# autonomousvision/LaRa

Hardware: AMD Instinct MI355X
Metric: novel-view frames/sec @512x512 (4-view in, 2DGS fwd+bwd) (higher is better)
Workload: dtype f32 raster + bf16-MFMA/f32-accumulate encoder (+ bf16-autocast coarse decoder MLP, as the reference's bf16-mixed)

## Files before the change

### lara_amd/csrc/abi.hip

```cpp
#include <stdlib.h>
#include <string.h>

#include "common.h"

static thread_local int g_last_hip_error = 0;
void l2d_set_hip_error(hipError_t e) { g_last_hip_error = (int)e; }

#include <atomic>
#include <mutex>
#include <map>
#include <utility>
#include <vector>
namespace {
struct ProfRec { const char *name; hipEvent_t a, b; };
std::atomic<bool> g_prof_on{false};
std::mutex g_prof_mu;
std::vector<ProfRec> g_prof_log;
std::vector<hipEvent_t> g_prof_pool;
hipEvent_t prof_event() {
    if (!g_prof_pool.empty()) { hipEvent_t e = g_prof_pool.back(); g_prof_pool.pop_back(); return e; }
    hipEvent_t e = nullptr;
    (void)hipEventCreate(&e);
    return e;
}
}

L2dProfScope::L2dProfScope(const char *name, hipStream_t stream) : slot(-1), s(stream) {
    if (!g_prof_on.load(std::memory_order_relaxed)) return;
    std::lock_guard<std::mutex> lk(g_prof_mu);
    ProfRec r{name, prof_event(), prof_event()};
    (void)hipEventRecord(r.a, s);
    g_prof_log.push_back(r);
    slot = (int)g_prof_log.size() - 1;
}
L2dProfScope::~L2dProfScope() {
    if (slot < 0) return;
    std::lock_guard<std::mutex> lk(g_prof_mu);
    if (slot < (int)g_prof_log.size()) (void)hipEventRecord(g_prof_log[slot].b, s);
}

namespace {

bool make_view(const lara2dgs_view *view, ViewDev &v) {
    if (!view) return false;
    if (view->P < 0 || view->image_height <= 0 || view->image_width <= 0) return false;
    if (view->sh_degree < 0 || view->sh_degree > 3) return false;
    if (view->capacity < 0 || view->capacity > 0xffffffffll) return false;
    if (!view->bg || !view->viewmatrix || !view->projmatrix || !view->campos) return false;
    v.P = view->P;
    v.deg = view->sh_degree;
    v.M = view->sh_coeffs;
    v.H = view->image_height;
    v.W = view->image_width;
    v.gx = (v.W + TILE - 1) / TILE;
    v.gy = (v.H + TILE - 1) / TILE;
    v.tiles = v.gx * v.gy;
    if (v.gx > 65535 || v.gy > 65535) return false;
    v.scale_modifier = view->scale_modifier;
    v.cull_transparent = (view->prefiltered >> 1) & 1;
    v.tight_tiles = (view->prefiltered >> 2) & 1;
    v.cap = (unsigned)view->capacity;
    v.fwd_only = view->forward_only != 0;
    v.counts_out = view->counts_out;
    {
        static const unsigned dbg = getenv("LARA2DGS_DEBUG_FLAGS") ? (unsigned)strtoul(getenv("LARA2DGS_DEBUG_FLAGS"), nullptr, 0) : 0u;
        v.dbg = dbg;
    }
    v.bg = view->bg;
    v.viewmatrix = view->viewmatrix;
    v.projmatrix = view->projmatrix;
    v.campos = view->campos;
    return true;
}

StateView carve_state(const ViewDev &v, void *state) {
    lara2dgs_state_layout L;
    state_layout(v.P, v.H, v.W, v.cap, v.fwd_only, &L);
    char *b = (char *)state;
    StateView s;
    s.header = (uint32_t *)(b + L.header);
    s.geom = (float4 *)(b + L.geom);
    s.cullbox = (float4 *)(b + L.cullbox);
    s.point_list = (uint32_t *)(b + L.point_list);
    s.ranges = (uint2 *)(b + L.ranges);
    s.tile_order = (uint32_t *)(b + L.tile_order);
    s.pair_base = (uint32_t *)(b + L.pair_base);
    s.pair_pos = (uint32_t *)(b + L.pair_pos);
    s.final_T = (float *)(b + L.final_T);
    s.n_contrib = (uint32_t *)(b + L.n_contrib);
    s.seg_base = (uint32_t *)(b + L.seg_base);
    s.seg_cnt = (uint32_t *)(b + L.seg_cnt);
    s.bwd_order = (uint32_t *)(b + L.bwd_order);
    s.bwd_items = (uint2 *)(b + L.bwd_items);
    s.ckpt = (float *)(b + L.ckpt);
    s.pair_mask = (uint2 *)(b + L.pair_mask);
    s.tile_maxc = (uint32_t *)(b + L.tile_maxc);
    s.seg_cost = (uint32_t *)(b + L.seg_cost);
    return s;
}

ScratchView carve_scratch(const ViewDev &v, void *scratch, ScratchLayout &L) {
    scratch_layout(v.P, v.H, v.W, v.cap, v.fwd_only, &L);
    char *b = (char *)scratch;
    ScratchView s;
    s.tile_count = (uint32_t *)(b + L.tile_count);
    s.tile_fill = (uint32_t *)(b + L.tile_fill);
    s.sub_start = (uint32_t *)(b + L.sub_start);
    s.sort_parts = (uint32_t *)(b + L.sort_parts);
    s.sort_items = (uint2 *)(b + L.sort_items);
    s.rect = (uint4 *)(b + L.rect);
    s.keys = (uint64_t *)(b + L.keys);
    s.block_tot = (uint32_t *)(b + L.block_tot);
    s.pair_grad = (float4 *)(b + L.pair_grad);
    s.pair_valid = (uint32_t *)(b + L.pair_valid);
    return s;
}

}

extern "C" {

int lara2dgs_abi_version(void) { return LARA2DGS_ABI_VERSION; }

const char *lara2dgs_error_string(int code) {
    switch (code) {
    case LARA2DGS_OK: return "ok";
    case LARA2DGS_E_INVALID: return "invalid argument";
    case LARA2DGS_E_LAUNCH: return "HIP launch/API failure (see lara2dgs_last_hip_error)";
    case LARA2DGS_E_UNSUPPORTED: return "unsupported configuration";
    default: return "unknown error";
    }
}

int lara2dgs_last_hip_error(void) { return g_last_hip_error; }

int64_t lara2dgs_state_bytes(int32_t P, int32_t H, int32_t W, int64_t capacity, int32_t forward_only) {
    if (P < 0 || H <= 0 || W <= 0 || capacity < 0) return LARA2DGS_E_INVALID;
    lara2dgs_state_layout L;
    state_layout(P, H, W, capacity, forward_only != 0, &L);
    return L.total;
}

int64_t lara2dgs_scratch_bytes(int32_t P, int32_t H, int32_t W, int64_t capacity, int32_t forward_only) {
    if (P < 0 || H <= 0 || W <= 0 || capacity < 0) return LARA2DGS_E_INVALID;
    ScratchLayout L;
    scratch_layout(P, H, W, capacity, forward_only != 0, &L);
    return L.total;
}

int lara2dgs_get_state_layout(int32_t P, int32_t H, int32_t W, int64_t capacity, int32_t forward_only,
                              lara2dgs_state_layout *out) {
    if (!out || P < 0 || H <= 0 || W <= 0 || capacity < 0) return LARA2DGS_E_INVALID;
    state_layout(P, H, W, capacity, forward_only != 0, out);
    return LARA2DGS_OK;
}

int lara2dgs_mark_visible(int32_t P, const float *means3D, const float *viewmatrix,
                          const float *projmatrix, uint8_t *present, void *stream) {
    (void)projmatrix;
    if (P < 0 || (P > 0 && (!means3D || !viewmatrix || !present))) return LARA2DGS_E_INVALID;
    return launch_mark_visible(P, means3D, viewmatrix, present, (hipStream_t)stream);
}

int lara2dgs_selftest(int which, const float *in, float *out, void *stream) {
    if (which != 0 || !in || !out) return LARA2DGS_E_INVALID;
    return launch_selftest_butterfly(in, out, (hipStream_t)stream);
}

int lara2dgs_profile_enable(int on) {
    g_prof_on.store(on != 0);
    return LARA2DGS_OK;
}

int lara2dgs_profile_collect(char *names, int names_len, float *ms, int max_entries) {
    std::lock_guard<std::mutex> lk(g_prof_mu);
    int n = 0, pos = 0;
    for (size_t i = 0; i < g_prof_log.size(); i++) {
        ProfRec &r = g_prof_log[i];
        if (n < max_entries && names && ms) {
            const int len = (int)strlen(r.name) + 1;
            if (pos + len <= names_len) {
                float t = 0.f;
                (void)hipEventSynchronize(r.b);
                (void)hipEventElapsedTime(&t, r.a, r.b);
                memcpy(names + pos, r.name, len);
                pos += len;
                ms[n++] = t;
            }
        }
        g_prof_pool.push_back(r.a);
        g_prof_pool.push_back(r.b);
    }
    g_prof_log.clear();
    return n;
}

}

namespace {

bool views_agree(int n, const lara2dgs_view *views) {
    for (int i = 1; i < n; i++) {
        const lara2dgs_view &a = views[0], &b = views[i];
        if (a.P != b.P || a.sh_degree != b.sh_degree || a.sh_coeffs != b.sh_coeffs || a.image_height != b.image_height ||
            a.image_width != b.image_width || a.capacity != b.capacity || a.prefiltered != b.prefiltered ||
            a.scale_modifier != b.scale_modifier || a.debug != b.debug || a.forward_only != b.forward_only) return false;
        if (b.counts_out != (a.counts_out ? a.counts_out + 4 * i : nullptr)) return false;
    }
    return true;
}

void grad_layout(int64_t P, int M, bool sh, bool col, bool sr, bool tm, lara2dgs_grad_layout *L) {
    int64_t o = 0;
    auto sec = [&](bool on, int64_t n) { if (!on) return (int64_t)-1; const int64_t at = o; o = (o + n + 3) / 4 * 4; return at; };
    L->means3D = sec(true, P * 3);
    L->means2D = sec(true, P * 3);
    L->shs = sec(sh, P * M * 3);
    L->colors = sec(col, P * 3);
    L->opacities = sec(true, P);
    L->scales = sec(sr, P * 2);
    L->rotations = sec(sr, P * 4);
    L->transmat = sec(tm, P * 9);
    L->total = o;
}

__global__ void __launch_bounds__(256) zero_strided_kernel(char *__restrict__ base, const int64_t stride, const int64_t bytes) {
    uint4 *p = (uint4 *)(base + (int64_t)blockIdx.y * stride);
    const int64_t n = bytes / 16;
    for (int64_t i = (int64_t)blockIdx.x * 256 + threadIdx.x; i < n; i += (int64_t)gridDim.x * 256) p[i] = make_uint4(0u, 0u, 0u, 0u);
}

inline int zero_strided(void *base, int64_t stride, int64_t bytes, int n_views, hipStream_t s) {
    const int64_t n = (bytes + 15) / 16;
    const unsigned gx = (unsigned)(n < 256 * 64 ? (n + 255) / 256 : 64);
    L2D_LAUNCH_IN_SCOPE(s, zero_strided_kernel, dim3(gx ? gx : 1, (unsigned)n_views), dim3(256), 0, (char *)base, stride, (bytes + 15) / 16 * 16);
    return LARA2DGS_OK;
}

bool strides_ok(const lara2dgs_view &v0, int64_t state_stride, int64_t scratch_stride) {
    return state_stride % 256 == 0 && scratch_stride % 256 == 0 &&
           state_stride >= lara2dgs_state_bytes(v0.P, v0.image_height, v0.image_width, v0.capacity, v0.forward_only) &&
           scratch_stride >= lara2dgs_scratch_bytes(v0.P, v0.image_height, v0.image_width, v0.capacity, v0.forward_only);
}

void one_view_strides(const lara2dgs_view &v, int64_t &state_stride, int64_t &scratch_stride) {
    state_stride = align_up(lara2dgs_state_bytes(v.P, v.image_height, v.image_width, v.capacity, v.forward_only), 256);
    scratch_stride = align_up(lara2dgs_scratch_bytes(v.P, v.image_height, v.image_width, v.capacity, v.forward_only), 256);
}
}

extern "C" {

int lara2dgs_get_grad_layout(int32_t P, int32_t sh_coeffs, int32_t has_shs, int32_t has_colors,
                             int32_t has_scale_rot, int32_t has_transmat, lara2dgs_grad_layout *out) {
    if (!out || P < 0 || sh_coeffs < 0) return LARA2DGS_E_INVALID;
    grad_layout(P, sh_coeffs, has_shs != 0, has_colors != 0, has_scale_rot != 0, has_transmat != 0, out);
    return LARA2DGS_OK;
}

static int forward_views_impl(int32_t n_views, const lara2dgs_view *views, const float *means3D,
                           const float *shs, const float *colors_precomp, const float *opacities,
                           const float *scales, const float *rotations, const float *transmat_precomp,
                           float *out_color, float *out_allmap, int32_t *out_radii, void *state,
                           int64_t state_stride, void *scratch, int64_t scratch_stride, void *stream,
                           const lara2dgs_subset *subset) {
    if (n_views <= 0 || !views || !state || !scratch) return LARA2DGS_E_INVALID;
    if (subset) {
        if (!subset->coarse_state || !subset->inv || subset->coarse_P < views[0].P || subset->coarse_capacity < 0 ||
            subset->coarse_capacity > 0xffffffffll || subset->coarse_state_stride % 256) return LARA2DGS_E_INVALID;
        if (!views[0].forward_only && subset->coarse_forward_only) return LARA2DGS_E_INVALID;
        if (subset->coarse_state_stride < lara2dgs_state_bytes(subset->coarse_P, views[0].image_height, views[0].image_width,
                                                                subset->coarse_capacity, subset->coarse_forward_only)) return LARA2DGS_E_INVALID;
    }
    if (!views_agree(n_views, views)) return LARA2DGS_E_INVALID;
    const lara2dgs_view &v0 = views[0];
    if (!strides_ok(v0, state_stride, scratch_stride)) return LARA2DGS_E_INVALID;
    hipStream_t caller = (hipStream_t)stream;
    const int64_t HW = (int64_t)v0.image_height * v0.image_width;
    if (!out_color || !out_allmap) return LARA2DGS_E_INVALID;
    if (v0.P > 0) {
        if (!means3D || !opacities || !out_radii) return LARA2DGS_E_INVALID;
        if ((shs == nullptr) == (colors_precomp == nullptr)) return LARA2DGS_E_INVALID;
        if ((scales && rotations) == (transmat_precomp != nullptr)) return LARA2DGS_E_INVALID;
    }
    std::vector<ViewDev> vd(n_views);
    std::vector<StateView> st(n_views);
    std::vector<ScratchView> sc(n_views);
    std::vector<int32_t *> rad(n_views);
    for (int i = 0; i < n_views; i++) {
        if (!make_view(&views[i], vd[i])) return LARA2DGS_E_INVALID;
        if (v0.P > 0 && shs && vd[i].M < (vd[i].deg + 1) * (vd[i].deg + 1)) return LARA2DGS_E_INVALID;
        st[i] = carve_state(vd[i], (char *)state + i * state_stride);
        ScratchLayout SL;
        sc[i] = carve_scratch(vd[i], (char *)scratch + i * scratch_stride, SL);
        rad[i] = out_radii + (int64_t)i * v0.P;
        if (i == 0)
            L2D_TRY(zero_strided(sc[0].tile_count, scratch_stride, SL.sub_start - SL.tile_count, n_views, caller));
    }
    int rc = LARA2DGS_OK;
    for (int i0 = 0; i0 < n_views && rc == LARA2DGS_OK; i0 += L2D_MAX_VIEWS) {
        ViewBatch vb{};
        vb.n = n_views - i0 < L2D_MAX_VIEWS ? n_views - i0 : L2D_MAX_VIEWS;
        vb.state_stride = state_stride; vb.scratch_stride = scratch_stride;
        for (int k = 0; k < vb.n; k++) vb.bg[k] = vd[i0 + k].bg;
        rc = launch_preprocess_fwd_views(vd[i0], vb.n, &vd[i0], n_views > 1, means3D, shs, colors_precomp, opacities, scales,
                                         rotations, transmat_precomp, &st[i0], &sc[i0], &rad[i0], caller);
        if (rc == LARA2DGS_OK && !subset) rc = launch_binning(vd[i0], st[i0], sc[i0], caller, vb);
        if (rc == LARA2DGS_OK && subset) {
            ViewDev cv = vd[i0];
            cv.P = subset->coarse_P; cv.cap = (unsigned)subset->coarse_capacity; cv.fwd_only = subset->coarse_forward_only != 0;
            const StateView cst = carve_state(cv, (char *)const_cast<void *>(subset->coarse_state) + (int64_t)i0 * subset->coarse_state_stride);
            rc = launch_binning_subset(vd[i0], st[i0], sc[i0], caller, vb, cst, subset->coarse_state_stride, subset->inv);
        }
        if (rc == LARA2DGS_OK)
            rc = launch_composite_fwd(vd[i0], st[i0], sc[i0], out_color + (int64_t)i0 * 3 * HW, out_allmap + (int64_t)i0 * 7 * HW,
                                      caller, vb);
    }
    return rc;
}

int lara2dgs_forward_views(int32_t n_views, const lara2dgs_view *views, const float *means3D,
                           const float *shs, const float *colors_precomp, const float *opacities,
                           const float *scales, const float *rotations, const float *transmat_precomp,
                           float *out_color, float *out_allmap, int32_t *out_radii, void *state,
                           int64_t state_stride, void *scratch, int64_t scratch_stride, void *stream) {
    return forward_views_impl(n_views, views, means3D, shs, colors_precomp, opacities, scales, rotations, transmat_precomp, out_color,
                              out_allmap, out_radii, state, state_stride, scratch, scratch_stride, stream, nullptr);
}

int lara2dgs_forward_views_subset(int32_t n_views, const lara2dgs_view *views, const float *means3D,
                                  const float *shs, const float *colors_precomp, const float *opacities,
                                  const float *scales, const float *rotations, const float *transmat_precomp,
                                  float *out_color, float *out_allmap, int32_t *out_radii, void *state,
                                  int64_t state_stride, void *scratch, int64_t scratch_stride,
                                  const lara2dgs_subset *subset, void *stream) {
    if (!subset) return LARA2DGS_E_INVALID;
    return forward_views_impl(n_views, views, means3D, shs, colors_precomp, opacities, scales, rotations, transmat_precomp, out_color,
                              out_allmap, out_radii, state, state_stride, scratch, scratch_stride, stream, subset);
}

static int backward_views_impl(int32_t n_views, const lara2dgs_view *views, const float *means3D, const float *shs,
                               const float *colors_precomp, const float *scales, const float *rotations,
                               const float *transmat_precomp, const int32_t *radii, const float *dL_dcolor,
                               const float *dL_dallmap, void *state, int64_t state_stride, void *scratch,
                               int64_t scratch_stride, float *dL_dmeans3D, float *dL_dmeans2D, float *dL_dshs,
                               float *dL_dcolors, float *dL_dopacities, float *dL_dscales, float *dL_drotations,
                               float *dL_dtransmat, void *stream) {
    const lara2dgs_view &v0 = views[0];
    hipStream_t caller = (hipStream_t)stream;
    const int64_t HW = (int64_t)v0.image_height * v0.image_width;
    std::vector<ViewDev> vd(n_views);
    std::vector<StateView> st(n_views);
    std::vector<ScratchView> sc(n_views);
    std::vector<const int32_t *> rad(n_views);
    std::vector<ScratchLayout> SL(n_views);
    for (int i = 0; i < n_views; i++) {
        if (!make_view(&views[i], vd[i])) return LARA2DGS_E_INVALID;
        st[i] = carve_state(vd[i], (char *)state + i * state_stride);
        sc[i] = carve_scratch(vd[i], (char *)scratch + i * scratch_stride, SL[i]);
        rad[i] = radii + (int64_t)i * v0.P;
    }
    int rc = LARA2DGS_OK;
    for (int i0 = 0; i0 < n_views && rc == LARA2DGS_OK; i0 += L2D_MAX_VIEWS) {
        ViewBatch vb{};
        vb.n = n_views - i0 < L2D_MAX_VIEWS ? n_views - i0 : L2D_MAX_VIEWS;
        vb.state_stride = state_stride; vb.scratch_stride = scratch_stride;
        for (int k = 0; k < vb.n; k++) vb.bg[k] = vd[i0 + k].bg;
        rc = launch_bwd_order(vd[i0], st[i0], sc[i0], caller, vb, sc[i0].pair_valid, SL[i0].total - SL[i0].pair_valid);
        if (rc == LARA2DGS_OK)
            rc = launch_composite_bwd(vd[i0], st[i0], sc[i0], dL_dcolor + (int64_t)i0 * 3 * HW, dL_dallmap ? dL_dallmap + (int64_t)i0 * 7 * HW : nullptr, caller, vb);
        if (rc == LARA2DGS_OK)
            rc = launch_preprocess_bwd_views(vd[i0], vb.n, &vd[i0], n_views > 1, i0 > 0, means3D, shs, colors_precomp, scales,
                                             rotations, transmat_precomp, &rad[i0], &st[i0], &sc[i0], dL_dmeans3D, dL_dmeans2D,
                                             dL_dshs, dL_dcolors, dL_dopacities, dL_dscales, dL_drotations, dL_dtransmat, caller);
    }
    return rc;
}

int lara2dgs_backward_views(int32_t n_views, const lara2dgs_view *views, const float *means3D,
                            const float *shs, const float *colors_precomp, const float *scales,
                            const float *rotations, const float *transmat_precomp, const int32_t *radii,
                            const float *dL_dcolor, const float *dL_dallmap, void *state,
                            int64_t state_stride, void *scratch, int64_t scratch_stride,
                            float *grad_out, void *stream) {
    if (n_views <= 0 || !views || !state || !scratch || !grad_out) return LARA2DGS_E_INVALID;
    if (!views_agree(n_views, views)) return LARA2DGS_E_INVALID;
    const lara2dgs_view &v0 = views[0];
    if (v0.forward_only) return LARA2DGS_E_INVALID;
    if (!strides_ok(v0, state_stride, scratch_stride)) return LARA2DGS_E_INVALID;
    if (!dL_dcolor) return LARA2DGS_E_INVALID;
    const bool has_sh = shs != nullptr, has_col = colors_precomp != nullptr, has_sr = scales && rotations,
               has_tm = transmat_precomp != nullptr;
    lara2dgs_grad_layout G;
    grad_layout(v0.P, v0.sh_coeffs, has_sh, has_col, has_sr, has_tm, &G);
    if (v0.P == 0 || G.total == 0) return LARA2DGS_OK;
    if (!means3D || !radii) return LARA2DGS_E_INVALID;
    if (has_sh == has_col || has_sr == has_tm) return LARA2DGS_E_INVALID;
    auto at = [&](int64_t off) { return off < 0 ? (float *)nullptr : grad_out + off; };
    return backward_views_impl(n_views, views, means3D, shs, colors_precomp, scales, rotations, transmat_precomp, radii,
                               dL_dcolor, dL_dallmap, state, state_stride, scratch, scratch_stride, at(G.means3D),
                               at(G.means2D), at(G.shs), at(G.colors), at(G.opacities), at(G.scales), at(G.rotations),
                               at(G.transmat), stream);
}

int lara2dgs_forward(const lara2dgs_view *view, const float *means3D, const float *shs,
                     const float *colors_precomp, const float *opacities, const float *scales,
                     const float *rotations, const float *transmat_precomp, float *out_color,
                     float *out_allmap, int32_t *out_radii, void *state, void *scratch,
                     void *stream) {
    ViewDev v;
    if (!make_view(view, v)) return LARA2DGS_E_INVALID;
    if (!out_color || !out_allmap || !state || !scratch) return LARA2DGS_E_INVALID;
    if (v.P > 0) {
        if (!means3D || !opacities || !out_radii) return LARA2DGS_E_INVALID;
        if ((shs == nullptr) == (colors_precomp == nullptr)) return LARA2DGS_E_INVALID;
        const bool has_sr = scales && rotations;
        if (has_sr == (transmat_precomp != nullptr)) return LARA2DGS_E_INVALID;
        if (shs && v.M < (v.deg + 1) * (v.deg + 1)) return LARA2DGS_E_INVALID;
    }
    int64_t sst, qst;
    one_view_strides(*view, sst, qst);
    return forward_views_impl(1, view, means3D, shs, colors_precomp, opacities, scales, rotations, transmat_precomp, out_color,
                              out_allmap, out_radii, state, sst, scratch, qst, stream, nullptr);
}

int lara2dgs_backward(const lara2dgs_view *view, const float *means3D, const float *shs,
                      const float *colors_precomp, const float *scales, const float *rotations,
                      const float *transmat_precomp, const int32_t *radii, const float *dL_dcolor,
                      const float *dL_dallmap, void *state, void *scratch,
                      float *dL_dmeans3D, float *dL_dmeans2D, float *dL_dshs, float *dL_dcolors,
                      float *dL_dopacities, float *dL_dscales, float *dL_drotations,
                      float *dL_dtransmat, void *stream) {
    ViewDev v;
    if (!make_view(view, v)) return LARA2DGS_E_INVALID;
    if (!dL_dcolor || !state || !scratch) return LARA2DGS_E_INVALID;
    if (v.fwd_only) return LARA2DGS_E_INVALID;
    if (v.P == 0) return LARA2DGS_OK;
    if (!means3D || !radii || !dL_dmeans3D || !dL_dmeans2D || !dL_dopacities) return LARA2DGS_E_INVALID;
    if ((shs == nullptr) == (colors_precomp == nullptr)) return LARA2DGS_E_INVALID;
    if (shs && !dL_dshs) return LARA2DGS_E_INVALID;
    if (colors_precomp && !dL_dcolors) return LARA2DGS_E_INVALID;
    const bool has_sr = scales && rotations;
    if (has_sr == (transmat_precomp != nullptr)) return LARA2DGS_E_INVALID;
    if (has_sr && (!dL_dscales || !dL_drotations)) return LARA2DGS_E_INVALID;
    if (transmat_precomp && !dL_dtransmat) return LARA2DGS_E_INVALID;
    int64_t sst, qst;
    one_view_strides(*view, sst, qst);
    return backward_views_impl(1, view, means3D, shs, colors_precomp, scales, rotations, transmat_precomp, radii, dL_dcolor,
                               dL_dallmap, state, sst, scratch, qst, dL_dmeans3D, dL_dmeans2D, dL_dshs, dL_dcolors,
                               dL_dopacities, dL_dscales, dL_drotations, dL_dtransmat, stream);
}

}
```

### lara_amd/csrc/common.h

```cpp
#pragma once
#include <hip/hip_runtime.h>
#include <stdint.h>

#include "../../include/lara2dgs.h"
#include "launch.h"

#define TILE 16
#define NEAR_N 0.2f
#define FAR_N 100.0f
#define FILTER_SIZE 0.707106f
#define FILTER_INV_SQUARE 2.0f
#define CUTOFF 3.0f
#define GEOM_F 20
#define L2D_SLICES 16
#define L2D_LDS_HIST_TILES 8192
#define GRAD_F 20
#define L2D_SEG 512
#define L2D_CKPT_F 10
#define L2D_MAX_VIEWS 8

struct ViewDev {
    int P, deg, M, H, W, gx, gy, tiles;
    float scale_modifier;
    unsigned cap;
    unsigned dbg;
    int cull_transparent;
    int tight_tiles;
    int fwd_only;
    const float *bg, *viewmatrix, *projmatrix, *campos;
    uint32_t *counts_out;
};

struct ViewBatch {
    int n;
    long long state_stride, scratch_stride;
    const float *bg[L2D_MAX_VIEWS];
};
#ifdef __HIPCC__
template <class T>
__device__ __forceinline__ T *l2d_view_ptr(T *p, const long long stride_bytes) {
    return (T *)((const char *)p + (long long)blockIdx.z * stride_bytes);
}
#endif

struct StateView {
    uint32_t *header;
    float4 *geom;
    float4 *cullbox;
    uint32_t *point_list;
    uint2 *ranges;
    uint32_t *tile_order;
    uint32_t *pair_base;
    uint32_t *pair_pos;
    float *final_T;
    uint32_t *n_contrib;
    uint32_t *seg_base;
    uint32_t *seg_cnt;
    uint32_t *bwd_order;
    uint2 *bwd_items;
    float *ckpt;
    uint2 *pair_mask;
    uint32_t *tile_maxc;
    uint32_t *seg_cost;
};

struct ScratchView {
    uint32_t *tile_count;
    uint32_t *tile_fill;
    uint32_t *sub_start;
    uint32_t *sort_parts;
    uint2 *sort_items;
    uint4 *rect;
    uint64_t *keys;
    uint32_t *block_tot;
    float4 *pair_grad;
    uint32_t *pair_valid;
};

static inline int64_t align_up(int64_t x, int64_t a) { return (x + a - 1) / a * a; }
static inline size_t up256(size_t v) { return (v + 255) & ~(size_t)255; }

__host__ __device__ static inline int64_t l2d_ckpt_slots(int64_t cap) { return cap / L2D_SEG + 1; }

static inline void state_layout(int P, int H, int W, int64_t cap, int fwd_only, lara2dgs_state_layout *L) {
    const int64_t tiles = (int64_t)((W + TILE - 1) / TILE) * ((H + TILE - 1) / TILE);
    const int64_t HW = (int64_t)H * W;
    const int64_t k = fwd_only ? 0 : 1;
    int64_t o = 0;
    L->header = o;      o = align_up(o + 256, 256);
    L->geom = o;        o = align_up(o + (int64_t)P * GEOM_F * 4, 256);
    L->cullbox = o;     o = align_up(o + (int64_t)P * 16, 256);
    L->point_list = o;  o = align_up(o + cap * 4, 256);
    L->ranges = o;      o = align_up(o + tiles * 8, 256);
    L->tile_order = o;  o = align_up(o + tiles * 4, 256);
    L->pair_base = o;   o = align_up(o + k * ((int64_t)P + 1) * 4, 256);
    L->pair_pos = o;    o = align_up(o + k * cap * 4, 256);
    L->final_T = o;     o = align_up(o + k * L2D_CKPT_F * HW * 4, 256);
    L->n_contrib = o;   o = align_up(o + k * 2 * HW * 4, 256);
    const int64_t nseg = cap / L2D_SEG + 1;
    L->seg_base = o;    o = align_up(o + k * (tiles + 1) * 4, 256);
    L->seg_cnt = o;     o = align_up(o + k * tiles * 4, 256);
    L->bwd_order = o;   o = align_up(o + k * tiles * 4, 256);
    L->bwd_items = o;   o = align_up(o + k * (nseg + tiles) * 8, 256);
    L->ckpt = o;        o = align_up(o + k * l2d_ckpt_slots(cap) * L2D_CKPT_F * 256 * 4, 256);
    L->pair_mask = o;   o = align_up(o + k * cap * 8, 256);
    L->tile_maxc = o;   o = align_up(o + k * tiles * 4, 256);
    L->seg_cost = o;    o = align_up(o + k * (nseg + tiles) * 4, 256);
    L->total = o;
}

struct ScratchLayout { int64_t tile_count, tile_fill, sub_start, sort_parts, sort_items, rect, keys, block_tot, pair_grad, pair_valid, total; };
static inline void scratch_layout(int P, int H, int W, int64_t cap, int fwd_only, ScratchLayout *L) {
    const int64_t tiles = (int64_t)((W + TILE - 1) / TILE) * ((H + TILE - 1) / TILE);
    int64_t o = 0;
    L->tile_count = o;  o = align_up(o + tiles * 4 * L2D_SLICES, 256);
    L->tile_fill = o;   o = align_up(o + tiles * 4 * L2D_SLICES, 256);
    L->sub_start = o;   o = align_up(o + tiles * 4 * L2D_SLICES, 256);
    L->sort_parts = o;  o = align_up(o + (tiles + 1) * 4, 256);
    L->sort_items = o;  o = align_up(o + tiles * 8, 256);
    const int64_t fwd0 = o;
    L->rect = o;        o = align_up(o + (int64_t)P * 16, 256);
    L->keys = o;        o = align_up(o + cap * 8, 256);
    L->block_tot = o;   o = align_up(o + (((int64_t)P + 255) / 256 + 1) * 4, 256);
    const int64_t fwd_end = o;
    L->pair_grad = fwd0;
    L->pair_valid = align_up(fwd0 + cap * GRAD_F * 4, 256);
    const int64_t bwd_end = align_up(L->pair_valid + cap + 256, 256);
    L->total = (fwd_only || fwd_end > bwd_end) ? fwd_end : bwd_end;
}

int launch_preprocess_fwd_views(const ViewDev &v, int n, const ViewDev *views, bool multi, const float *means3D, const float *shs,
                                const float *colors_precomp, const float *opacities, const float *scales,
                                const float *rotations, const float *transmat_precomp, const StateView *st,
                                const ScratchView *sc, int32_t *const *radii, hipStream_t s);
int launch_binning(const ViewDev &v, StateView st, ScratchView sc, hipStream_t s, const ViewBatch &vb);
int launch_binning_subset(const ViewDev &v, StateView st, ScratchView sc, hipStream_t s, const ViewBatch &vb, StateView cst,
                          long long coarse_stride, const int32_t *inv);
int launch_composite_fwd(const ViewDev &v, StateView st, ScratchView sc, float *out_color, float *out_allmap,
                         hipStream_t s, const ViewBatch &vb);
int launch_bwd_order(const ViewDev &v, StateView st, ScratchView sc, hipStream_t s, const ViewBatch &vb, void *zero_base, int64_t zero_bytes);
int launch_composite_bwd(const ViewDev &v, StateView st, ScratchView sc, const float *dL_dcolor,
                         const float *dL_dallmap, hipStream_t s, const ViewBatch &vb);
int launch_preprocess_bwd_views(const ViewDev &v, int n, const ViewDev *views, bool multi, int accumulate, const float *means3D,
                                const float *shs, const float *colors_precomp, const float *scales, const float *rotations,
                                const float *transmat_precomp, const int32_t *const *radii, const StateView *st,
                                const ScratchView *sc, float *dL_dmeans3D, float *dL_dmeans2D, float *dL_dshs,
                                float *dL_dcolors, float *dL_dopacities, float *dL_dscales, float *dL_drotations,
                                float *dL_dtransmat, hipStream_t s);
int launch_selftest_butterfly(const float *in, float *out, hipStream_t s);
int launch_mark_visible(int P, const float *means3D, const float *viewmatrix, uint8_t *present,
                        hipStream_t s);
```

### lara_amd/csrc/composite.hip

```cpp
#include "common.h"
#include "tilebox.h"
#include "wave.h"

namespace {

constexpr int FWD_CHUNK = 512;
constexpr int REC4 = 6;

__device__ __forceinline__ void cross3(const float a[3], const float b[3], float o[3]) {
    o[0] = a[1] * b[2] - a[2] * b[1];
    o[1] = a[2] * b[0] - a[0] * b[2];
    o[2] = a[0] * b[1] - a[1] * b[0];
}

template <int CHUNK>
__device__ __forceinline__ uint32_t stage_entry(const float4 *__restrict__ geom, const uint32_t id,
                                                const float4 cb, const bool valid, const float X0,
                                                const float Y0, float4 *rec, uint32_t *ids,
                                                const int e = threadIdx.x, uint2 *mask_out = nullptr) {
    float4 r0 = make_float4(0.f, 0.f, 0.f, 0.f), r1 = r0, r2 = r0, r3 = r0, r4 = r0, r5 = r0;
    uint32_t mask_lo = 0, mask_hi = 0, rectpack = 0;
    int gx0 = 0, gx1 = -1, gy0 = 0, gy1 = -1;
    if (valid) {
        l2d_box_cells<2>(cb.x, cb.y, X0, 8.f, gx0, gx1);
        l2d_box_cells<2>(cb.z, cb.w, Y0, 8.f, gy0, gy1);
    }
    if (gx0 <= gx1 && gy0 <= gy1) {
        const float4 *g = geom + (size_t)id * 5;
        const float4 g0 = g[0], g1 = g[1], g2 = g[2], g3 = g[3], g4 = g[4];
        const float Tu[3] = {g0.x, g0.y, g0.z}, Tv[3] = {g0.w, g1.x, g1.y}, Tw[3] = {g1.z, g1.w, g2.x};
        const float k0[3] = {X0 * Tw[0] - Tu[0], X0 * Tw[1] - Tu[1], X0 * Tw[2] - Tu[2]};
        const float l0[3] = {Y0 * Tw[0] - Tv[0], Y0 * Tw[1] - Tv[1], Y0 * Tw[2] - Tv[2]};
        float A[3], B[3], C[3];
        cross3(k0, l0, A);
        cross3(Tw, l0, B);
        cross3(k0, Tw, C);
        const float cx = g2.y - X0, cy = g2.z - Y0, opa = g2.w;
        const float tau = 2.0f * __logf(255.0f * opa) * 1.001f + 0.01f;
        const float nb = B[0] * B[0] + B[1] * B[1], qa = nb - tau * B[2] * B[2];
        const bool ellipse = qa > 1e-5f * (nb + tau * B[2] * B[2]);
        const float inv_qa = ellipse ? __builtin_amdgcn_rcpf(qa) : 0.f;
        const float bx0 = (float)(2 * gx0), bx1 = (float)(2 * gx1 + 1);
        uint32_t colsum = 0;
        for (int by = gy0; by <= gy1; by++) {
            float lo = 1e9f, hi = -1e9f;
#pragma unroll
            for (int q = 0; q < 2; q++) {
                const float y = (float)(2 * by + q);
                const float u0 = A[0] + y * C[0], u1 = A[1] + y * C[1], u2 = A[2] + y * C[2];
                const float qb = u0 * B[0] + u1 * B[1] - tau * (u2 * B[2]);
                const float qc = u0 * u0 + u1 * u1 - tau * (u2 * u2);
                const float disc = qb * qb - qa * qc + 4e-6f * (qb * qb);
                if (!ellipse) {
                    lo = bx0; hi = bx1;
                } else if (disc >= 0.f) {
                    const float sq = __builtin_amdgcn_sqrtf(disc);
                    lo = fminf(lo, (-qb - sq) * inv_qa);
                    hi = fmaxf(hi, (-qb + sq) * inv_qa);
                }
                const float h = 0.5f * tau - (y - cy) * (y - cy);
                if (h >= 0.f) {
                    const float sh = __builtin_amdgcn_sqrtf(h);
                    lo = fminf(lo, cx - sh);
                    hi = fmaxf(hi, cx + sh);
                }
            }
            const int ilo = (int)ceilf(fmaxf(lo - 0.02f, bx0)), ihi = (int)floorf(fminf(hi + 0.02f, bx1));
            if (ilo <= ihi) {
                const uint32_t cols = ((2u << (ihi >> 1)) - 1u) & ~((1u << (ilo >> 1)) - 1u);
                colsum |= cols;
                if (by < 4) mask_lo |= cols << (8 * by);
                else mask_hi |= cols << (8 * (by - 4));
            }
        }
        if (colsum) {
            const int rx0 = __builtin_ctz(colsum), rx1 = 31 - __builtin_clz(colsum);
            const int ry0 = mask_lo ? (__builtin_ctz(mask_lo) >> 3) : 4 + (__builtin_ctz(mask_hi) >> 3);
            const int ry1 = mask_hi ? 4 + ((31 - __builtin_clz(mask_hi)) >> 3) : ((31 - __builtin_clz(mask_lo)) >> 3);
            rectpack = (uint32_t)rx0 | ((uint32_t)rx1 << 4) | ((uint32_t)ry0 << 8) | ((uint32_t)ry1 << 12) | (1u << 16);
            r0 = make_float4(A[0], A[1], A[2], B[0]);
            r1 = make_float4(B[1], B[2], C[0], C[1]);
            r2 = make_float4(C[2], cx, cy, Tw[0]);
            r3 = make_float4(Tw[1], Tw[2], opa, __uint_as_float(mask_lo));
            r4 = make_float4(g3.x, g3.y, g3.z, g4.x);
            r5 = make_float4(g4.y, g4.z, __uint_as_float(mask_hi), 0.f);
        }
    }
    rec[0 * CHUNK + e] = r0; rec[1 * CHUNK + e] = r1; rec[2 * CHUNK + e] = r2;
    rec[3 * CHUNK + e] = r3; rec[4 * CHUNK + e] = r4; rec[5 * CHUNK + e] = r5;
    if (ids) ids[e] = valid ? id : 0u;
    if (mask_out && valid) *mask_out = make_uint2(mask_lo, mask_hi);
    return rectpack;
}

template <int CHUNK>
__device__ __forceinline__ void stage_entry_masked(const float4 *__restrict__ geom, const uint32_t id, const uint2 mask,
                                                   const bool valid, const float X0, const float Y0, float4 *rec,
                                                   uint32_t *ids, const int e) {
    float4 r0 = make_float4(0.f, 0.f, 0.f, 0.f), r1 = r0, r2 = r0, r3 = r0, r4 = r0, r5 = r0;
    if (valid && (mask.x | mask.y)) {
        const float4 *g = geom + (size_t)id * 5;
        const float4 g0 = g[0], g1 = g[1], g2 = g[2], g3 = g[3], g4 = g[4];
        const float Tu[3] = {g0.x, g0.y, g0.z}, Tv[3] = {g0.w, g1.x, g1.y}, Tw[3] = {g1.z, g1.w, g2.x};
        const float k0[3] = {X0 * Tw[0] - Tu[0], X0 * Tw[1] - Tu[1], X0 * Tw[2] - Tu[2]};
        const float l0[3] = {Y0 * Tw[0] - Tv[0], Y0 * Tw[1] - Tv[1], Y0 * Tw[2] - Tv[2]};
        float A[3], B[3], C[3];
        cross3(k0, l0, A);
        cross3(Tw, l0, B);
        cross3(k0, Tw, C);
        r0 = make_float4(A[0], A[1], A[2], B[0]);
        r1 = make_float4(B[1], B[2], C[0], C[1]);
        r2 = make_float4(C[2], g2.y - X0, g2.z - Y0, Tw[0]);
        r3 = make_float4(Tw[1], Tw[2], g2.w, __uint_as_float(mask.x));
        r4 = make_float4(g3.x, g3.y, g3.z, g4.x);
        r5 = make_float4(g4.y, g4.z, __uint_as_float(mask.y), 0.f);
    }
    rec[0 * CHUNK + e] = r0; rec[1 * CHUNK + e] = r1; rec[2 * CHUNK + e] = r2;
    rec[3 * CHUNK + e] = r3; rec[4 * CHUNK + e] = r4; rec[5 * CHUNK + e] = r5;
    ids[e] = valid ? id : 0u;
}

struct Hit {
    float sx, sy, rz, depth, G, alpha, ddx, ddy;
    bool use3d;
};

struct EntryRec { float4 r0, r1, r2, r3; };
template <int CHUNK>
__device__ __forceinline__ EntryRec load_entry(const float4 *rec, const int j) {
    EntryRec e;
    e.r0 = rec[0 * CHUNK + j]; e.r1 = rec[1 * CHUNK + j]; e.r2 = rec[2 * CHUNK + j]; e.r3 = rec[3 * CHUNK + j];
    return e;
}

__device__ __forceinline__ bool eval_rec(const EntryRec &e, const float lx, const float ly, Hit &h,
                                         float Tw[3], float &opa) {
    const float4 r0 = e.r0, r1 = e.r1, r2 = e.r2, r3 = e.r3;
    const float px = r0.x + lx * r0.w + ly * r1.z;
    const float py = r0.y + lx * r1.x + ly * r1.w;
    const float pz = r0.z + lx * r1.y + ly * r2.x;
    Tw[0] = r2.w; Tw[1] = r3.x; Tw[2] = r3.y; opa = r3.z;
    h.rz = __builtin_amdgcn_rcpf(pz);
    h.sx = px * h.rz; h.sy = py * h.rz;
    const float rho3d = h.sx * h.sx + h.sy * h.sy;
    h.ddx = r2.y - lx; h.ddy = r2.z - ly;
    const float rho2d = FILTER_INV_SQUARE * (h.ddx * h.ddx + h.ddy * h.ddy);
    h.use3d = rho3d <= rho2d;
    const float rho = fminf(rho3d, rho2d);
    h.depth = h.use3d ? (h.sx * Tw[0] + h.sy * Tw[1]) + Tw[2] : Tw[2];
    const float power = -0.5f * rho;
    h.G = __expf(power);
    h.alpha = fminf(0.99f, opa * h.G);
    return (pz != 0.0f) & (h.depth >= NEAR_N) & !(power > 0.0f) & !(h.alpha < 1.0f / 255.0f);
}

__device__ __forceinline__ unsigned long long quad_masks(const uint32_t bm, const int qx4, const int grp) {
    unsigned long long m = 0ull;
#pragma unroll
    for (int g = 0; g < 16; g++) {
        const int bit = (g >> 2) * 8 + qx4 + (g & 3);
        const unsigned long long b = __ballot((bm >> bit) & 1u);
        m = (grp == g) ? b : m;
    }
    return m;
}

struct FwdPixel {
    float T = 1.0f, C0 = 0.f, C1 = 0.f, C2 = 0.f, N0 = 0.f, N1 = 0.f, N2 = 0.f;
    float Dd = 0.f, M1 = 0.f, M2 = 0.f, distortion = 0.f, median_depth = 0.f;
    uint32_t last_contributor = 0, median_contributor = 0;
    bool done = false;

    template <int CHUNK>
    __device__ __forceinline__ void blend(const float4 *rec, const int j, const int base, bool valid,
                                          const Hit &h) {
        valid = valid && !done;
        const float test_T = T * (1.0f - h.alpha);
        const bool kill = valid && test_T < 0.0001f;
        done = done || kill;
        valid = valid && !kill;
        if (__ballot(valid) == 0ull) return;
        const float4 r4 = rec[4 * CHUNK + j], r5 = rec[5 * CHUNK + j];
        const float a = valid ? h.alpha : 0.f;
        const float depth = valid ? h.depth : 1.0f;
        const float w = a * T;
        const float A = 1.0f - T;
        const float mm = FAR_N / (FAR_N - NEAR_N) * (1.0f - NEAR_N * __builtin_amdgcn_rcpf(depth));
        distortion += (mm * mm * A + M2 - 2.0f * mm * M1) * w;
        Dd += depth * w;
        M1 += mm * w;
        M2 += mm * mm * w;
        const bool med = valid && T > 0.5f;
        median_depth = med ? depth : median_depth;
        median_contributor = med ? (uint32_t)(base + j + 1) : median_contributor;
        N0 += r4.x * w; N1 += r4.y * w; N2 += r4.z * w;
        C0 += r4.w * w; C1 += r5.x * w; C2 += r5.y * w;
        T = valid ? test_T : T;
        last_contributor = valid ? (uint32_t)(base + j + 1) : last_contributor;
    }

};

template <bool KEEP>
__global__ void __launch_bounds__(256)
composite_fwd_kernel(ViewDev v, const uint32_t *__restrict__ header, const uint2 *__restrict__ ranges,
                     const uint32_t *__restrict__ point_list, const float4 *__restrict__ geom,
                     const uint32_t *__restrict__ tile_order, const float4 *__restrict__ cullbox,
                     float *__restrict__ final_T, uint32_t *__restrict__ n_contrib,
                     const uint32_t *__restrict__ seg_base, const uint32_t *__restrict__ seg_cnt,
                     float *__restrict__ ckpt, uint2 *__restrict__ pair_mask, uint32_t *__restrict__ tile_maxc,
                     uint32_t *__restrict__ seg_cost,
                     float *__restrict__ out_color, float *__restrict__ out_allmap, const ViewBatch vb) {
    {
        const long long sst = vb.state_stride, HWb = (long long)v.H * v.W * 4;
        header = l2d_view_ptr(header, sst); ranges = l2d_view_ptr(ranges, sst); point_list = l2d_view_ptr(point_list, sst);
        geom = l2d_view_ptr(geom, sst); tile_order = l2d_view_ptr(tile_order, sst); cullbox = l2d_view_ptr(cullbox, sst);
        final_T = l2d_view_ptr(final_T, sst); n_contrib = l2d_view_ptr(n_contrib, sst); seg_base = l2d_view_ptr(seg_base, sst);
        seg_cnt = l2d_view_ptr(seg_cnt, sst); ckpt = l2d_view_ptr(ckpt, sst); pair_mask = l2d_view_ptr(pair_mask, sst);
        tile_maxc = l2d_view_ptr(tile_maxc, sst); seg_cost = l2d_view_ptr(seg_cost, sst);
        out_color = l2d_view_ptr(out_color, 3 * HWb); out_allmap = l2d_view_ptr(out_allmap, 7 * HWb);
        v.bg = vb.bg[blockIdx.z];
    }
    constexpr int CHUNK = FWD_CHUNK;
    static_assert(L2D_SEG % FWD_CHUNK == 0, "segment boundaries must fall on round boundaries");
    __shared__ float4 rec[REC4 * CHUNK];
    __shared__ unsigned long long qmask[4][16][CHUNK / 64];
    uint32_t &s_cost = *(uint32_t *)&rec[5 * CHUNK + 0].w;
    uint32_t &s_tmax = *(uint32_t *)&rec[5 * CHUNK + 1].w;
    uint32_t &s_ndone = *(uint32_t *)&rec[5 * CHUNK + 2].w;
    const int tile = (v.dbg & 8u) ? (int)blockIdx.x : (int)tile_order[blockIdx.x];
    const int tx = tile % v.gx, ty = tile / v.gx;
    const int wave = threadIdx.x >> 6, lane = threadIdx.x & 63;
    const int grp = lane >> 2;
    const int lxi = (wave & 1) * 8 + (grp & 3) * 2 + (lane & 1);
    const int lyi = (wave >> 1) * 8 + (grp >> 2) * 2 + ((lane >> 1) & 1);
    const int pxi = tx * TILE + lxi, pyi = ty * TILE + lyi;
    const bool inside = pxi < v.W && pyi < v.H;
    const size_t HW = (size_t)v.H * v.W;
    const size_t pix = (size_t)pyi * v.W + pxi;
    const float lx = (float)lxi, ly = (float)lyi;
    const float X0 = (float)(tx * TILE), Y0 = (float)(ty * TILE);

    if (header[1]) {
        if (inside) {
            const float qnan = __uint_as_float(0x7fc00000u);
            for (int ch = 0; ch < 3; ch++) out_color[ch * HW + pix] = qnan;
            for (int ch = 0; ch < 7; ch++) out_allmap[ch * HW + pix] = qnan;
            if (KEEP) {
                for (int ch = 0; ch < L2D_CKPT_F; ch++) final_T[pix + ch * HW] = qnan;
                n_contrib[pix] = 0; n_contrib[pix + HW] = 0;
            }
        }
        return;
    }

    const uint2 range = ranges[tile];
    const int total = (int)(range.y - range.x);
    const int lo = 0, hi = total;
    FwdPixel px;
    px.done = !inside;
    uint32_t *dbg_hdr = const_cast<uint32_t *>(header);
    const long long dbg_t0 = (v.dbg & 32u) ? (long long)__builtin_readcyclecounter() : 0ll;
    int dbg_rounds = 0;

    const int tid = threadIdx.x;
    const uint32_t cost_nb = KEEP ? seg_cnt[tile] : 0u;
    uint32_t *const cost_full = KEEP ? seg_cost + seg_base[tile] : nullptr,
             *const cost_last = KEEP ? seg_cost + (v.cap / L2D_SEG + 1u) + tile : nullptr;
    if (KEEP)
        for (uint32_t q = tid; q <= cost_nb; q += 256) *(q < cost_nb ? cost_full + q : cost_last) = 0u;
    int cost_round = -1;
    constexpr int SPT = CHUNK / 256;
    uint32_t id1[SPT], id2[SPT];
    float4 cb1[SPT];
#pragma unroll
    for (int q = 0; q < SPT; q++) {
        const int o = lo + q * 256 + tid;
        id1[q] = o < hi ? point_list[range.x + o] : 0u;
        id2[q] = CHUNK + o < hi ? point_list[range.x + CHUNK + o] : 0u;
    }
#pragma unroll
    for (int q = 0; q < SPT; q++) cb1[q] = lo + q * 256 + tid < hi ? cullbox[id1[q]] : make_float4(0.f, 0.f, 0.f, 0.f);
    if (threadIdx.x < 3) *(uint32_t *)&rec[5 * CHUNK + threadIdx.x].w = 0u;
    __syncthreads();
    for (int base = lo; base < hi; base += CHUNK) {
        {
            const bool wave_done = __ballot(px.done) == ~0ull;
            if (wave_done && lane == 0) atomicAdd(&s_ndone, 1u);
            __syncthreads();
            if (s_ndone == 4u) break;
        }
        if (KEEP && tid == 0) {
            if (cost_round >= 0) { if ((uint32_t)cost_round < cost_nb) cost_full[cost_round] = s_cost; else *cost_last += s_cost; }
            s_cost = 0u;
        }
        cost_round = (base - lo) / CHUNK;
        dbg_rounds++;
        if (KEEP && base && base % L2D_SEG == 0 && !px.done) {
            float *ck = ckpt + ((size_t)seg_base[tile] + (size_t)(base / L2D_SEG - 1)) * (L2D_CKPT_F * 256) + tid;
            ck[0 * 256] = px.T; ck[1 * 256] = px.M1; ck[2 * 256] = px.M2;
            ck[3 * 256] = px.C0; ck[4 * 256] = px.C1; ck[5 * 256] = px.C2;
            ck[6 * 256] = px.Dd; ck[7 * 256] = px.N0; ck[8 * 256] = px.N1; ck[9 * 256] = px.N2;
        }
#pragma unroll
        for (int q = 0; q < SPT; q++) {
            const int o = q * 256 + tid;
            const uint32_t id0 = id1[q];
            const float4 cb0 = cb1[q];
            id1[q] = id2[q];
            id2[q] = base + 2 * CHUNK + o < hi ? point_list[range.x + base + 2 * CHUNK + o] : 0u;
            cb1[q] = base + CHUNK + o < hi ? cullbox[id1[q]] : make_float4(0.f, 0.f, 0.f, 0.f);
            stage_entry<CHUNK>(geom, id0, cb0, base + o < hi, X0, Y0, rec, nullptr, o,
                               KEEP && base + o < hi ? pair_mask + range.x + base + o : nullptr);
        }
        __syncthreads();
        if (__ballot(!px.done) == 0ull) continue;
        const int nw = (min(CHUNK, hi - base) + 63) >> 6;
        unsigned long long *qm = &qmask[wave][grp][0];
#pragma unroll 1
        for (int w = 0; w < nw; w++) {
            const float4 *mrec = rec + ((wave >> 1) ? 5 : 3) * CHUNK + w * 64 + lane;
            const uint32_t bm = __float_as_uint((wave >> 1) ? mrec->z : mrec->w);
            unsigned long long m = 0ull;
            if (__ballot((bm & (0x0f0f0f0fu << ((wave & 1) * 4))) != 0u) != 0ull) m = quad_masks(bm, (wave & 1) * 4, grp);
            if ((lane & 3) == 0) qm[w] = m;
        }
        int w = 0;
        unsigned long long mm = qm[0];
        if (((__ballot(px.done) >> (lane & ~3)) & 0xfull) == 0xfull) { mm = 0ull; w = nw; }
        auto next = [&](bool &has, int &j) {
            while (mm == 0ull && w + 1 < nw) { w++; mm = qm[w]; }
            has = mm != 0ull;
            j = has ? 64 * w + __builtin_ctzll(mm) : 0;
            mm &= mm - 1ull;
        };
        bool hA0, hA1, hB0 = false, hB1 = false;
        int jA0, jA1, jB0 = 0, jB1 = 0;
        next(hA0, jA0);
        next(hA1, jA1);
        EntryRec rA0 = load_entry<CHUNK>(rec, jA0), rA1 = load_entry<CHUNK>(rec, jA1), rB0, rB1;
        auto trip = [&](const EntryRec &c0, const EntryRec &c1, const int j0, const int j1, const bool has0, const bool has1,
                        EntryRec &x0, EntryRec &x1, int &k0, int &k1, bool &n0, bool &n1) {
            next(n0, k0);
            next(n1, k1);
            x0 = load_entry<CHUNK>(rec, k0);
            x1 = load_entry<CHUNK>(rec, k1);
            Hit h0, h1;
            float Tw0[3], Tw1[3], opa0, opa1;
            const bool e0 = eval_rec(c0, lx, ly, h0, Tw0, opa0) && has0;
            const bool e1 = eval_rec(c1, lx, ly, h1, Tw1, opa1) && has1;
            if (v.dbg & 4u) {
                atomicAdd(&dbg_hdr[4], ((lane & 3) == 0) ? (unsigned)has0 + (unsigned)has1 : 0u);
                atomicAdd(&dbg_hdr[5], (unsigned)e0 + (unsigned)e1);
                if (lane == 0) atomicAdd(&dbg_hdr[6], 1u);
            }
            px.blend<CHUNK>(rec, j0, base, e0, h0);
            px.blend<CHUNK>(rec, j1, base, e1, h1);
            if (((__ballot(px.done) >> (lane & ~3)) & 0xfull) == 0xfull) { mm = 0ull; w = nw; n0 = false; n1 = false; }
        };
        uint32_t ntrips = 0;
        while (true) {
            if (__ballot(hA0) == 0ull) break;
            trip(rA0, rA1, jA0, jA1, hA0, hA1, rB0, rB1, jB0, jB1, hB0, hB1);
            ntrips++;
            if (__ballot(hB0) == 0ull) break;
            trip(rB0, rB1, jB0, jB1, hB0, hB1, rA0, rA1, jA0, jA1, hA0, hA1);
            ntrips++;
        }
        if (KEEP && lane == 0 && ntrips) atomicAdd(&s_cost, ntrips);
    }
    const float T = px.T;
    if (KEEP) {
        if (threadIdx.x == 0) s_tmax = 0u;
        __syncthreads();
        uint32_t m = px.last_contributor;
#pragma unroll
        for (int d = 1; d < 64; d <<= 1) m = max(m, (uint32_t)__shfl_xor((int)m, d, 64));
        if (lane == 0) atomicMax(&s_tmax, m);
        __syncthreads();
        if (threadIdx.x == 0) {
            tile_maxc[tile] = s_tmax;
            if (cost_round >= 0) { if ((uint32_t)cost_round < cost_nb) cost_full[cost_round] = s_cost; else *cost_last += s_cost; }
        }
    }
    if (inside) {
        if (KEEP) {
            final_T[pix] = T;
            final_T[pix + HW] = px.M1;
            final_T[pix + 2 * HW] = px.M2;
            final_T[pix + 3 * HW] = px.C0; final_T[pix + 4 * HW] = px.C1; final_T[pix + 5 * HW] = px.C2;
            final_T[pix + 6 * HW] = px.Dd;
            final_T[pix + 7 * HW] = px.N0; final_T[pix + 8 * HW] = px.N1; final_T[pix + 9 * HW] = px.N2;
            n_contrib[pix] = px.last_contributor;
            n_contrib[pix + HW] = px.median_contributor;
        }
        out_color[0 * HW + pix] = px.C0 + T * v.bg[0];
        out_color[1 * HW + pix] = px.C1 + T * v.bg[1];
        out_color[2 * HW + pix] = px.C2 + T * v.bg[2];
        out_allmap[0 * HW + pix] = px.Dd;
        out_allmap[1 * HW + pix] = 1.0f - T;
        out_allmap[2 * HW + pix] = px.N0;
        out_allmap[3 * HW + pix] = px.N1;
        out_allmap[4 * HW + pix] = px.N2;
        out_allmap[5 * HW + pix] = px.median_depth;
        out_allmap[6 * HW + pix] = px.distortion;
        if ((v.dbg & 32u) && lane == 0) {
            out_allmap[6 * HW + pix] = (float)((long long)__builtin_readcyclecounter() - dbg_t0);
            out_allmap[5 * HW + pix] = (float)dbg_rounds;
        }
    }
}

__device__ __forceinline__ float mul_legacy(const float a, const float b) {
    float r;
    asm("v_mul_legacy_f32 %0, %1, %2" : "=v"(r) : "v"(a), "v"(b));
    return r;
}

struct QuadCoef { float a1, a2, a3, b1, b2, b3; };
__device__ __forceinline__ QuadCoef quad_coef(const int lane, const float lx, const float ly) {
    QuadCoef k;
    const int l = lane & 3;
    k.a1 = l == 0 ? 1.f : (l == 1 ? lx - 1.f : (l == 2 ? ly : 0.f));
    k.a2 = l == 1 ? 1.f : 0.f;
    k.a3 = l == 3 ? 1.f : 0.f;
    k.b1 = l == 0 ? ly : (l == 2 ? 1.f : (l == 3 ? lx - 1.f : 0.f));
    k.b2 = l == 3 ? 1.f : 0.f;
    k.b3 = l == 1 ? 1.f : 0.f;
    return k;
}
__device__ __forceinline__ void quad_reduce_scatter(const float dp[3], const float q[3], const float h[10], const QuadCoef &k,
                                                    float r[6], const int lane) {
    const bool b0 = lane & 1, b1 = lane & 2;
#pragma unroll
    for (int c = 0; c < 3; c++) {
        float d = dp[c];
        asm volatile("" : "+v"(d));
        const float t = d + dpp_move<0xB1, 0xf>(d);
        const float tq = q[c] + dpp_move<0xB1, 0xf>(q[c]);
        const float mine = k.a1 * t + (k.a2 * d + k.a3 * tq);
        const float send = k.b1 * t + (k.b2 * d + k.b3 * tq);
        r[c] = mine + dpp_move<0x4E, 0xf>(send);
    }
    float v1[5];
#pragma unroll
    for (int i = 0; i < 5; i++) {
        const float mine = b0 ? h[2 * i + 1] : h[2 * i];
        const float send = b0 ? h[2 * i] : h[2 * i + 1];
        v1[i] = mine + dpp_move<0xB1, 0xf>(send);
    }
#pragma unroll
    for (int i = 0; i < 2; i++) {
        const float mine = b1 ? v1[2 * i + 1] : v1[2 * i];
        const float send = b1 ? v1[2 * i] : v1[2 * i + 1];
        r[3 + i] = mine + dpp_move<0x4E, 0xf>(send);
    }
    r[5] = v1[4] + dpp_move<0x4E, 0xf>(v1[4]);
}
__device__ __forceinline__ void quad_reduce_scatter16(const float dp[3], const float q[3], const float h[4], const QuadCoef &k,
                                                      float r[4], const int lane) {
    const bool b0 = lane & 1, b1 = lane & 2;
#pragma unroll
    for (int c = 0; c < 3; c++) {
        float d = dp[c], qq = q[c];
        asm volatile("" : "+v"(d));
        asm volatile("" : "+v"(qq));
        const float t = d + dpp_move<0xB1, 0xf>(d);
        const float tq = qq + dpp_move<0xB1, 0xf>(qq);
        const float mine = k.a1 * t + (k.a2 * d + k.a3 * tq);
        const float send = k.b1 * t + (k.b2 * d + k.b3 * tq);
        r[c] = mine + dpp_move<0x4E, 0xf>(send);
    }
    float v1[2];
#pragma unroll
    for (int i = 0; i < 2; i++) {
        const float mine = b0 ? h[2 * i + 1] : h[2 * i];
        const float send = b0 ? h[2 * i] : h[2 * i + 1];
        v1[i] = mine + dpp_move<0xB1, 0xf>(send);
    }
    const float mine = b1 ? v1[1] : v1[0];
    const float send = b1 ? v1[0] : v1[1];
    r[3] = mine + dpp_move<0x4E, 0xf>(send);
}

constexpr int SLAB_WIN = 128;
constexpr int SLAB_CHUNK = 128;
constexpr int SLAB_POOL = 374;
constexpr int SLAB_F = 24;
constexpr int SLAB_F_COLOR = 16;
constexpr int SLAB_POOL_COLOR = SLAB_POOL * SLAB_F / SLAB_F_COLOR;

template <bool MAPS>
__global__ void __launch_bounds__(256)
composite_bwd_kernel(ViewDev v, const uint32_t *__restrict__ header, const uint2 *__restrict__ ranges,
                     const uint32_t *__restrict__ point_list, const float4 *__restrict__ geom,
                     const uint32_t *__restrict__ tile_order, const float4 *__restrict__ cullbox,
                     const float *__restrict__ final_T, const uint32_t *__restrict__ n_contrib,
                     const uint32_t *__restrict__ seg_base, const uint32_t *__restrict__ seg_cnt,
                     const uint32_t *__restrict__ bwd_order,
                     const uint2 *__restrict__ bwd_items, const float *__restrict__ ckpt,
                     const uint2 *__restrict__ pair_mask, const uint32_t *__restrict__ tile_maxc,
                     const float *__restrict__ dL_dcolor, const float *__restrict__ dL_dallmap,
                     const uint32_t *__restrict__ pair_pos,
                     float4 *__restrict__ pair_grad, uint8_t *__restrict__ pair_valid, const ViewBatch vb) {
    {
        const long long sst = vb.state_stride, qst = vb.scratch_stride, HWb = (long long)v.H * v.W * 4;
        header = l2d_view_ptr(header, sst); ranges = l2d_view_ptr(ranges, sst); point_list = l2d_view_ptr(point_list, sst);
        geom = l2d_view_ptr(geom, sst); tile_order = l2d_view_ptr(tile_order, sst); cullbox = l2d_view_ptr(cullbox, sst);
        final_T = l2d_view_ptr(final_T, sst); n_contrib = l2d_view_ptr(n_contrib, sst); seg_base = l2d_view_ptr(seg_base, sst);
        seg_cnt = l2d_view_ptr(seg_cnt, sst); bwd_order = l2d_view_ptr(bwd_order, sst); bwd_items = l2d_view_ptr(bwd_items, sst);
        ckpt = l2d_view_ptr(ckpt, sst); pair_mask = l2d_view_ptr(pair_mask, sst); pair_pos = l2d_view_ptr(pair_pos, sst);
        tile_maxc = l2d_view_ptr(tile_maxc, sst);
        pair_grad = l2d_view_ptr(pair_grad, qst); pair_valid = l2d_view_ptr(pair_valid, qst);
        dL_dcolor = l2d_view_ptr(dL_dcolor, 3 * HWb); dL_dallmap = l2d_view_ptr(dL_dallmap, 7 * HWb);
        v.bg = vb.bg[blockIdx.z];
    }
    constexpr int WIN = SLAB_WIN;
    constexpr int POOL = MAPS ? SLAB_POOL : SLAB_POOL_COLOR, SF = MAPS ? SLAB_F : SLAB_F_COLOR;
    __shared__ float4 rec[REC4 * WIN];
    __shared__ __attribute__((aligned(16))) float pool[(POOL + 1) * SF];
    __shared__ uint16_t s_base_[2][SLAB_CHUNK];
    __shared__ unsigned long long s_live_[2][SLAB_CHUNK];
    __shared__ uint32_t s_ql[64];
    __shared__ uint32_t s_id_[2][WIN];
    __shared__ uint2 s_mask[WIN];
    __shared__ int s_nfit_[2];
    __shared__ uint32_t s_total_[2];
    if (header[1]) return;
    const unsigned long long dbg_t0 = (v.dbg & 32u) ? wall_clock64() : 0ull;
    int dbg_rounds = 0;
    uint32_t dbg_windows = 0, dbg_trips = 0, dbg_entries = 0, dbg_slots = 0, dbg_rows = 0;
    unsigned long long dbg_tp = 0ull;
    uint32_t dbg_ph[5] = {0u, 0u, 0u, 0u, 0u};
#define DBG_PHASE(k) do { if (v.dbg & 64u) { const unsigned long long t__ = __builtin_readcyclecounter(); dbg_ph[k] += (uint32_t)(t__ - dbg_tp); dbg_tp = t__; } } while (0)
    if (v.dbg & 64u) dbg_tp = __builtin_readcyclecounter();
    const uint32_t n_full = header[3];
    int tile, seg;
    if (header[22]) {
        if (blockIdx.x >= n_full + (uint32_t)v.tiles) return;
        const uint2 it = bwd_items[blockIdx.x];
        tile = (int)it.x; seg = (int)it.y;
    } else if (blockIdx.x < n_full) {
        const uint2 it = bwd_items[blockIdx.x];
        tile = (int)it.x; seg = (int)it.y;
    } else if (blockIdx.x - n_full < (uint32_t)v.tiles) {
        tile = (int)bwd_order[blockIdx.x - n_full];
        seg = (int)seg_cnt[tile];
    } else {
        return;
    }
    const uint2 range = ranges[tile];
    const int seg_lo = seg * L2D_SEG;
    const int seg_hi = seg == (int)seg_cnt[tile] ? (int)(range.y - range.x) : seg_lo + L2D_SEG;
    const int total = min((int)tile_maxc[tile], seg_hi);
    const int lo = seg_lo;
    if (total <= lo) return;
    const int tx = tile % v.gx, ty = tile / v.gx;
    const int tid = threadIdx.x, wave = tid >> 6, lane = tid & 63;
    const int grp = lane >> 2;
    const int lxi = (wave & 1) * 8 + (grp & 3) * 2 + (lane & 1);
    const int lyi = (wave >> 1) * 8 + (grp >> 2) * 2 + ((lane >> 1) & 1);
    const int pxi = tx * TILE + lxi, pyi = ty * TILE + lyi;
    const bool inside = pxi < v.W && pyi < v.H;
    const size_t HW = (size_t)v.H * v.W;
    const size_t pix = inside ? (size_t)pyi * v.W + pxi : 0;
    const float lx = (float)lxi, ly = (float)lyi;
    const float X0 = (float)(tx * TILE), Y0 = (float)(ty * TILE);

    const float T_final = inside ? final_T[pix] : 0.f;
    float T = T_final;
    const uint32_t last_contributor = inside ? n_contrib[pix] : 0u;
    const uint32_t median_contributor = (MAPS && inside) ? n_contrib[pix + HW] : 0u;
    float dpix[3] = {0.f, 0.f, 0.f}, dnrm[3] = {0.f, 0.f, 0.f};
    float dL_ddepth = 0.f, dL_daccum = 0.f, dL_dmedian = 0.f, dL_dreg = 0.f;
    float final_D = 0.f, final_D2 = 0.f;
    if (inside) {
        for (int ch = 0; ch < 3; ch++) dpix[ch] = dL_dcolor[ch * HW + pix];
        if constexpr (MAPS) {
            dL_ddepth = dL_dallmap[0 * HW + pix];
            dL_daccum = dL_dallmap[1 * HW + pix];
            for (int ch = 0; ch < 3; ch++) dnrm[ch] = dL_dallmap[(2 + ch) * HW + pix];
            dL_dmedian = dL_dallmap[5 * HW + pix];
            dL_dreg = dL_dallmap[6 * HW + pix];
            final_D = final_T[pix + HW];
            final_D2 = final_T[pix + 2 * HW];
        }
    }
    const float final_A = 1.0f - T_final;
    const float bg_dot_dpixel = v.bg[0] * dpix[0] + v.bg[1] * dpix[1] + v.bg[2] * dpix[2];

    float accum_g = 0.f, last_g = 0.f, last_alpha = 0.f;
    float last_dL_dT = 0.f;

    const int my_blk = (lyi >> 1) * 8 + (lxi >> 1);
    const uint32_t below_lo = my_blk >= 32 ? 0xffffffffu : (1u << my_blk) - 1u;
    const uint32_t below_hi = my_blk >= 32 ? (1u << (my_blk - 32)) - 1u : 0u;
    const QuadCoef qcoef = quad_coef(lane, lx, ly);
    uint32_t quad_last = last_contributor;
    quad_last = max(quad_last, (uint32_t)__builtin_amdgcn_update_dpp(0, (int)quad_last, 0xB1, 0xf, 0xf, false));
    quad_last = max(quad_last, (uint32_t)__builtin_amdgcn_update_dpp(0, (int)quad_last, 0x4E, 0xf, 0xf, false));
    if ((lane & 3) == 0) s_ql[my_blk] = quad_last;
    if (tid < SF) pool[POOL * SF + tid] = 0.f;

    if ((int)last_contributor > seg_hi) {
        const float *ck = ckpt + ((size_t)seg_base[tile] + (size_t)seg) * (L2D_CKPT_F * 256) + tid;
        const float Tb = ck[0], inv_Tb = 1.0f / Tb;
        T = Tb;
        const float s_alpha = (Tb - T_final) * inv_Tb;
        if constexpr (MAPS) {
            const float s_m1 = (final_D - ck[1 * 256]) * inv_Tb, s_m2 = (final_D2 - ck[2 * 256]) * inv_Tb;
            float sg = (Tb - T_final) * dL_daccum + (final_T[pix + 6 * HW] - ck[6 * 256]) * dL_ddepth;
            for (int ch = 0; ch < 3; ch++)
                sg += (final_T[pix + (3 + ch) * HW] - ck[(3 + ch) * 256]) * dpix[ch] +
                      (final_T[pix + (7 + ch) * HW] - ck[(7 + ch) * 256]) * dnrm[ch];
            accum_g = sg * inv_Tb;
            last_dL_dT = (final_D2 * s_alpha + final_A * s_m2 - 2.0f * final_D * s_m1) * dL_dreg;
        } else {
            (void)s_alpha;
            float sg = 0.f;
            for (int ch = 0; ch < 3; ch++) {
                float p = (final_T[pix + (3 + ch) * HW] - ck[(3 + ch) * 256]) * dpix[ch];
                asm volatile("" : "+v"(p));
                sg += p;
            }
            accum_g = sg * inv_Tb;
        }
    }

    const int se = tid - 128;
    const bool stager = se >= 0;
    uint32_t id1 = 0u, id2 = 0u;
    uint2 mk1 = make_uint2(0u, 0u), mk2 = mk1;
    auto size_round = [&](const int whi_, const int wcnt_, const int s0_, const int buf, const bool side) {
        unsigned long long *const live_ = s_live_[buf];
        uint16_t *const base_ = s_base_[buf];
                const int jm = max(whi_ - s0_ - (int)s_ql[lane], 0);
                unsigned long long la = ~0ull, lb = ~0ull;
                if (__ballot(jm > 0) != 0ull) {
                    volatile unsigned long long *vlive = live_;
                    vlive[2 * lane] = 0ull;
                    vlive[2 * lane + 1] = 0ull;
                    if (jm < SLAB_CHUNK) atomicOr(&live_[jm], 1ull << lane);
                    __builtin_amdgcn_wave_barrier();
                    la = vlive[2 * lane];
                    lb = la | vlive[2 * lane + 1];
                    unsigned long long ex = lb;
#pragma unroll
                    for (int d = 1; d < 64; d <<= 1) {
                        const uint32_t ylo = __shfl_up((uint32_t)ex, d, 64), yhi = __shfl_up((uint32_t)(ex >> 32), d, 64);
                        if (lane >= d) ex |= ((unsigned long long)yhi << 32) | ylo;
                    }
                    const uint32_t plo = __shfl_up((uint32_t)ex, 1, 64), phi = __shfl_up((uint32_t)(ex >> 32), 1, 64);
                    const unsigned long long before = lane ? (((unsigned long long)phi << 32) | plo) : 0ull;
                    la |= before; lb |= before;
                }
                uint32_t c[2];
#pragma unroll
                for (int q = 0; q < 2; q++) {
                    const int slot = s0_ + 2 * lane + q;
                    unsigned long long mk = 0ull;
                    if (slot < wcnt_) {
                        const uint2 mw = side ? s_mask[slot] : make_uint2(__float_as_uint(rec[3 * WIN + slot].w), __float_as_uint(rec[5 * WIN + slot].z));
                        mk = (((unsigned long long)mw.y << 32) | mw.x) & (q ? lb : la);
                    }
                    live_[2 * lane + q] = mk;
                    c[q] = (uint32_t)__builtin_popcountll(mk);
                }
                uint32_t incl = c[0] + c[1];
#pragma unroll
                for (int d = 1; d < 64; d <<= 1) {
                    const uint32_t y = __shfl_up(incl, d, 64);
                    if (lane >= d) incl += y;
                }
                const uint32_t b0 = incl - c[0] - c[1], b1 = incl - c[1];
                const unsigned long long f0 = __ballot(s0_ + 2 * lane < wcnt_ && b1 <= (uint32_t)POOL);
                const unsigned long long f1 = __ballot(s0_ + 2 * lane + 1 < wcnt_ && incl <= (uint32_t)POOL);
                const int L = f1 == ~0ull ? 64 : __builtin_ctzll(~f1);
                if (lane == 0) s_nfit_[buf] = L == 64 ? 128 : 2 * L + (int)((f0 >> L) & 1ull);
                base_[2 * lane] = (uint16_t)b0;
                base_[2 * lane + 1] = (uint16_t)b1;
                if (lane == 63) s_total_[buf] = incl;
    };
    {
        const int wcnt = min(WIN, total - lo);
        if (stager) {
            const uint32_t id0 = total - 1 - se >= lo ? point_list[range.x + total - 1 - se] : 0u;
            const uint2 mk0 = total - 1 - se >= lo ? pair_mask[range.x + total - 1 - se] : make_uint2(0u, 0u);
            id1 = total - WIN - 1 - se >= lo ? point_list[range.x + total - WIN - 1 - se] : 0u;
            mk1 = total - WIN - 1 - se >= lo ? pair_mask[range.x + total - WIN - 1 - se] : make_uint2(0u, 0u);
            id2 = total - 2 * WIN - 1 - se >= lo ? point_list[range.x + total - 2 * WIN - 1 - se] : 0u;
            mk2 = total - 2 * WIN - 1 - se >= lo ? pair_mask[range.x + total - 2 * WIN - 1 - se] : make_uint2(0u, 0u);
            stage_entry_masked<WIN>(geom, id0, mk0, se < wcnt, X0, Y0, rec, s_id_[0], se);
        }
        __syncthreads();
        if (wave == 3) size_round(total, wcnt, 0, 0, false);
        __syncthreads();
        DBG_PHASE(0);
    }
    int cur = 0, wb = 0;
    for (int whi = total; whi > lo; whi -= WIN) {
        const int wcnt = min(WIN, whi - lo);
        const bool more_windows = whi - WIN > lo;
        dbg_windows++;
        if (stager) s_mask[se] = mk1;
        unsigned long long wm0 = 0ull, wm1 = 0ull;

        for (int s0 = 0; s0 < wcnt;) {
            dbg_rounds++;
            const unsigned long long *const s_live = s_live_[cur];
            const uint16_t *const s_base = s_base_[cur];
            const uint32_t *const s_id = s_id_[wb];
            const int nfit = s_nfit_[cur];
            if (v.dbg & 512u) { dbg_entries += (uint32_t)nfit; dbg_slots += nfit < SLAB_CHUNK ? (uint32_t)s_base[nfit] : min(s_total_[cur], (uint32_t)POOL); }

            {
                if (s0 == 0) {
#pragma unroll
                    for (int k = 0; k < 2; k++) {
                        const float4 *mrec = rec + ((wave >> 1) ? 5 : 3) * WIN + 64 * k + lane;
                        const uint32_t bm = __float_as_uint((wave >> 1) ? mrec->z : mrec->w);
                        unsigned long long m = 0ull;
                        if (__ballot((bm & (0x0f0f0f0fu << ((wave & 1) * 4))) != 0u) != 0ull) m = quad_masks(bm, (wave & 1) * 4, grp);
                        if (k == 0) wm0 = m; else wm1 = m;
                    }
                }
                unsigned long long m0 = wm0, m1 = wm1;
                {
                    int sh = s0;
                    if (sh >= 64) { m0 = m1; m1 = 0ull; sh -= 64; }
                    if (sh) { m0 = (m0 >> sh) | (m1 << (64 - sh)); m1 >>= sh; }
                    if (nfit < 64) { m0 &= (1ull << nfit) - 1ull; m1 = 0ull; }
                    else if (nfit < 128) m1 &= (1ull << (nfit - 64)) - 1ull;
                }
                const int jmin = whi - s0 - (int)quad_last;
                if (jmin > 0) {
                    m0 = jmin >= 64 ? 0ull : m0 & (~0ull << jmin);
                    m1 = jmin >= 128 ? 0ull : (jmin > 64 ? m1 & (~0ull << (jmin - 64)) : m1);
                }
                uint32_t mm = (uint32_t)m0, q1 = (uint32_t)(m0 >> 32), q2 = (uint32_t)m1, q3 = (uint32_t)(m1 >> 32);
                int jb = 0;
                auto trip = [&]() __attribute__((always_inline)) {
                    dbg_trips++;
                    while (mm == 0u && (q1 | q2 | q3) != 0u) { mm = q1; q1 = q2; q2 = q3; q3 = 0u; jb += 32; }
                    const bool has = mm != 0u;
                    const int j = jb + (has ? __builtin_ctz(mm) : 0);
                    mm &= mm - 1u;
                    const int ws = s0 + j;
                    const uint32_t contributor = (uint32_t)(whi - 1 - ws);
                    const EntryRec ent = load_entry<WIN>(rec, ws);
                    Hit h;
                    float Tw[3], opa;
                    const bool active = eval_rec(ent, lx, ly, h, Tw, opa) && has && contributor < last_contributor;
                    const float4 r4 = rec[4 * WIN + ws], r5 = rec[5 * WIN + ws];
                    const float nrm[3] = {r4.x, r4.y, r4.z}, rgb[3] = {r4.w, r5.x, r5.y};
                    if constexpr (!MAPS) {
                        (void)nrm;
                        const float alpha = active ? h.alpha : 0.f;
                        const float inv_1ma = __builtin_amdgcn_rcpf(1.f - alpha);
                        const float T_new = T * inv_1ma;
                        const float w = alpha * T_new;
                        const float gval = __builtin_fmaf(rgb[2], dpix[2], __builtin_fmaf(rgb[0], dpix[0], rgb[1] * dpix[1]));
                        const float accum_new = mul_legacy(last_alpha, last_g) + (1.f - last_alpha) * accum_g;
                        float dL_dalpha = gval - accum_new;
                        dL_dalpha = __builtin_fmaf(T_new, dL_dalpha, -((T_final * inv_1ma) * bg_dot_dpixel));
                        T = T_new;
                        accum_g = accum_new;
                        last_g = gval;
                        last_alpha = alpha;
                        const float da = active ? dL_dalpha : 0.f;
                        const float sx = h.sx, sy = h.sy;
                        const float rz3 = (active && h.use3d) ? h.rz : 0.f;
                        const float qG = opa * da * h.G;
                        const float dL_dsx = -mul_legacy(qG, sx), dL_dsy = -mul_legacy(qG, sy);
                        const float dpx = dL_dsx * rz3, dpy = dL_dsy * rz3;
                        const float dpv[3] = {dpx, dpy, -(mul_legacy(dpx, sx) + mul_legacy(dpy, sy))};
                        const float qG2 = h.use3d ? 0.f : -FILTER_INV_SQUARE * qG;
                        const float q3[3] = {h.G * da, qG2 * h.ddx, qG2 * h.ddy};
                        const float h4[4] = {w * dpix[0], w * dpix[1], w * dpix[2], w};
                        float r[4];
                        quad_reduce_scatter16(dpv, q3, h4, qcoef, r, lane);
#pragma unroll
                        for (int i = 0; i < 4; i++) asm volatile("" : "+v"(r[i]));
                        const unsigned long long lv = s_live[has ? j : 0];
                        const int rank = __builtin_popcount((uint32_t)lv & below_lo) + __builtin_popcount((uint32_t)(lv >> 32) & below_hi);
                        float4 *ps = (float4 *)(pool + ((int)s_base[has ? j : 0] + rank) * SF) + (lane & 3);
                        if (has) *ps = make_float4(r[0], r[1], r[2], r[3]);
                    } else {
                    const float alpha = active ? h.alpha : 0.f, c_d = h.depth;
                    const float inv_1ma = __builtin_amdgcn_rcpf(1.f - alpha);
                    const float T_new = T * inv_1ma;
                    const float w = alpha * T_new;
                    const float gval = rgb[0] * dpix[0] + rgb[1] * dpix[1] + rgb[2] * dpix[2] +
                                       nrm[0] * dnrm[0] + nrm[1] * dnrm[1] + nrm[2] * dnrm[2] +
                                       c_d * dL_ddepth + dL_daccum;
                    const float accum_new = mul_legacy(last_alpha, last_g) + (1.f - last_alpha) * accum_g;
                    float dL_dalpha = gval - accum_new;
                    float dL_dz = 0.0f;
                    const float inv_cd = __builtin_amdgcn_rcpf(c_d);
                    const float m_d = FAR_N / (FAR_N - NEAR_N) * (1.f - NEAR_N * inv_cd);
                    const float dmd_dd = (FAR_N * NEAR_N) / (FAR_N - NEAR_N) * inv_cd * inv_cd;
                    if (contributor + 1 == median_contributor) dL_dz += dL_dmedian;
                    const float dL_dweight = (final_D2 + m_d * m_d * final_A - 2.f * m_d * final_D) * dL_dreg;
                    dL_dalpha += dL_dweight - last_dL_dT;
                    const float dLdT_new = mul_legacy(alpha, dL_dweight) + (1.f - alpha) * last_dL_dT;
                    const float dL_dmd = 2.0f * (T_new * alpha) * (m_d * final_A - final_D) * dL_dreg;
                    dL_dz += dL_dmd * dmd_dd;
                    dL_dalpha *= T_new;
                    dL_dalpha += (-T_final * inv_1ma) * bg_dot_dpixel;
                    dL_dz += w * dL_ddepth;
                    T = T_new;
                    accum_g = accum_new;
                    last_g = gval;
                    last_alpha = alpha;
                    last_dL_dT = dLdT_new;
                    const float ww = w, da = active ? dL_dalpha : 0.f, dz = active ? dL_dz : 0.f;
                    const float sx = h.sx, sy = h.sy;
                    const float rz3 = (active && h.use3d) ? h.rz : 0.f;
                    const float qv[3] = {mul_legacy(dz, sx), mul_legacy(dz, sy), dz};
                    const float qG = opa * da * h.G;
                    const float dL_dsx = dz * Tw[0] - mul_legacy(qG, sx);
                    const float dL_dsy = dz * Tw[1] - mul_legacy(qG, sy);
                    const float dpx = dL_dsx * rz3, dpy = dL_dsy * rz3;
                    const float dpv[3] = {dpx, dpy, -(mul_legacy(dpx, sx) + mul_legacy(dpy, sy))};
                    const float qG2 = h.use3d ? 0.f : -FILTER_INV_SQUARE * qG;
                    const float hv[10] = {qG2 * h.ddx, qG2 * h.ddy, ww * dnrm[0], ww * dnrm[1], ww * dnrm[2], h.G * da,
                                          ww * dpix[0], ww * dpix[1], ww * dpix[2], ww};
                    float r[6];
                    quad_reduce_scatter(dpv, qv, hv, qcoef, r, lane);
#pragma unroll
                    for (int i = 0; i < 6; i++) asm volatile("" : "+v"(r[i]));
                    const unsigned long long lv = s_live[has ? j : 0];
                    const int rank = __builtin_popcount((uint32_t)lv & below_lo) + __builtin_popcount((uint32_t)(lv >> 32) & below_hi);
                    float *ps = pool + ((int)s_base[has ? j : 0] + rank) * SLAB_F + (lane & 3);
                    if (has) {
                        ps[0] = r[0]; ps[4] = r[1]; ps[8] = r[2]; ps[12] = r[3]; ps[16] = r[4];
                        if (!(lane & 2)) ps[20] = r[5];
                    }
                    }
                };
                while (__ballot((mm | q1 | q2 | q3) != 0u) != 0ull) {
                    trip();
                    if (__ballot((mm | q1 | q2 | q3) != 0u) == 0ull) break;
                    trip();
                }
            }
            __syncthreads();
            DBG_PHASE(3);

            if ((wave << 5) < nfit && !(v.dbg & 2u)) {
                const int e = tid >> 1, part = tid & 1;
                const int ws = min(s0 + e, WIN - 1);
                const bool has = e < nfit;
                const int cnt = has ? __builtin_popcountll(s_live[e]) : 0;
                float4 gq0 = make_float4(0.f, 0.f, 0.f, 0.f), gq1 = gq0, gq2 = gq0;
                if (cnt && part == 0) {
                    const float4 *gm = geom + (size_t)s_id[ws] * 5;
                    gq0 = gm[0]; gq1 = gm[1]; gq2 = gm[2];
                }
                constexpr int NG = MAPS ? 22 : 16;
                float g[NG];
                const float4 *ps = (const float4 *)(pool + (int)s_base[e] * SF);
                {
                    const float4 *p0 = part < cnt ? ps + part * (SF / 4) : (const float4 *)(pool + POOL * SF);
#pragma unroll
                    for (int q = 0; q < NG / 4; q++) {
                        const float4 t = p0[q];
                        g[4 * q] = t.x; g[4 * q + 1] = t.y; g[4 * q + 2] = t.z; g[4 * q + 3] = t.w;
                    }
                    if constexpr (MAPS) {
                        const float2 t2 = *(const float2 *)(p0 + 5);
                        g[20] = t2.x; g[21] = t2.y;
                    }
                }
                for (int i = part + 2; i < cnt; i += 2) {
#pragma unroll
                    for (int q = 0; q < NG / 4; q++) {
                        const float4 t = ps[i * (SF / 4) + q];
                        g[4 * q] += t.x; g[4 * q + 1] += t.y; g[4 * q + 2] += t.z; g[4 * q + 3] += t.w;
                    }
                    if constexpr (MAPS) {
                        const float2 t2 = *(const float2 *)(ps + i * (SF / 4) + 5);
                        g[20] += t2.x; g[21] += t2.y;
                    }
                }
#pragma unroll
                for (int k = 0; k < NG; k++) g[k] += dpp_move<0xB1, 0xf>(g[k]);
                const bool touched = (MAPS ? g[21] : g[15]) > 0.f;
                if (part == 0 && touched) {
                    const uint32_t p = range.x + (uint32_t)(whi - 1 - ws);
                    const float4 g0 = gq0, g1 = gq1, g2 = gq2;
                    const float Tu[3] = {g0.x, g0.y, g0.z}, Tv[3] = {g0.w, g1.x, g1.y}, Tw[3] = {g1.z, g1.w, g2.x};
                    const float k0[3] = {X0 * Tw[0] - Tu[0], X0 * Tw[1] - Tu[1], X0 * Tw[2] - Tu[2]};
                    const float l0[3] = {Y0 * Tw[0] - Tv[0], Y0 * Tw[1] - Tv[1], Y0 * Tw[2] - Tv[2]};
                    const float a[3] = {g[0], MAPS ? g[4] : g[1], MAPS ? g[8] : g[2]};
                    const float b[3] = {MAPS ? g[1] : g[4], g[5], MAPS ? g[9] : g[6]};
                    const float cc[3] = {MAPS ? g[2] : g[8], MAPS ? g[6] : g[9], g[10]};
                    const float qd[3] = {MAPS ? g[3] : 0.f, MAPS ? g[7] : 0.f, MAPS ? g[11] : 0.f};
                    float t1[3], t2[3], dk0[3], dl0[3], dTw[3];
                    cross3(l0, a, t1); cross3(Tw, cc, t2);
                    for (int i = 0; i < 3; i++) dk0[i] = t1[i] + t2[i];
                    cross3(a, k0, t1); cross3(b, Tw, t2);
                    for (int i = 0; i < 3; i++) dl0[i] = t1[i] + t2[i];
                    cross3(l0, b, t1); cross3(cc, k0, t2);
                    for (int i = 0; i < 3; i++) {
                        dTw[i] = t1[i] + t2[i] + X0 * dk0[i] + Y0 * dl0[i];
                        if constexpr (MAPS) dTw[i] += qd[i];
                    }
                    const uint32_t q = pair_pos[p];
                    float4 *row = pair_grad + (size_t)q * (GRAD_F / 4);
                    row[0] = make_float4(-dk0[0], -dk0[1], -dk0[2], -dl0[0]);
                    row[1] = make_float4(-dl0[1], -dl0[2], dTw[0], dTw[1]);
                    if constexpr (MAPS) {
                        row[2] = make_float4(dTw[2], g[12], g[13], g[14]);
                        row[3] = make_float4(g[15], g[16], g[17], g[18]);
                        row[4] = make_float4(g[19], g[20], 0.f, 0.f);
                    } else {
                        row[2] = make_float4(dTw[2], g[13], g[14], 0.f);
                        row[3] = make_float4(0.f, 0.f, g[12], g[3]);
                        row[4] = make_float4(g[7], g[11], 0.f, 0.f);
                    }
                    pair_valid[q] = 1;
                    dbg_rows++;
                }
            }
            const bool last_round = s0 + nfit >= wcnt;
            if (stager && last_round && more_windows) {
                stage_entry_masked<WIN>(geom, id1, mk1, se < min(WIN, whi - WIN - lo), X0, Y0, rec, s_id_[wb ^ 1], se);
                id1 = id2;
                mk1 = mk2;
                id2 = whi - 3 * WIN - 1 - se >= lo ? point_list[range.x + whi - 3 * WIN - 1 - se] : 0u;
                mk2 = whi - 3 * WIN - 1 - se >= lo ? pair_mask[range.x + whi - 3 * WIN - 1 - se] : make_uint2(0u, 0u);
            }
            if (wave == 3) {
                if (!last_round) size_round(whi, wcnt, s0 + nfit, cur ^ 1, false);
                else if (more_windows) size_round(whi - WIN, min(WIN, whi - WIN - lo), 0, cur ^ 1, true);
            }
            __syncthreads();
            DBG_PHASE(4);
            s0 += nfit;
            cur ^= 1;
        }
        wb ^= 1;
    }
    if ((v.dbg & 64u) && tid == 0) {
        DBG_PHASE(4);
        uint32_t *h = const_cast<uint32_t *>(header);
        for (int k = 0; k < 5; k++) atomicAdd(&h[16 + k], dbg_ph[k] >> 6);
    }
    if (v.dbg & 512u) {
        uint32_t *h = const_cast<uint32_t *>(header);
        if (tid == 0) {
            atomicAdd(&h[24], 1u); atomicAdd(&h[25], dbg_windows); atomicAdd(&h[26], (uint32_t)dbg_rounds);
            atomicAdd(&h[28], dbg_entries); atomicAdd(&h[29], dbg_slots);
        }
        if (lane == 0) atomicAdd(&h[27], dbg_trips);
        if (dbg_rows) atomicAdd(&h[30], dbg_rows);
    }
    if ((v.dbg & 32u) && tid == 0) {
        uint32_t *h = const_cast<uint32_t *>(header);
        const unsigned long long t1 = wall_clock64();
        atomicMax(&h[8], (uint32_t)(t1 - dbg_t0));
        atomicMax((unsigned long long *)&h[12], ((unsigned long long)(uint32_t)(t1 - dbg_t0) << 32) |
                                                    ((unsigned long long)dbg_rounds << 16) | (unsigned long long)blockIdx.x);
        atomicAdd(&h[9], (uint32_t)(t1 - dbg_t0));
        atomicMax(&h[10], ~(uint32_t)dbg_t0);
        atomicMax(&h[11], (uint32_t)t1);
    }
}

__global__ void __launch_bounds__(64)
selftest_butterfly_kernel(const float *__restrict__ in, float *__restrict__ out) {
    const int lane = threadIdx.x, q4 = lane & 3, grp = lane >> 2;
    const float lx = (float)((grp & 3) * 2 + (lane & 1)), ly = (float)((grp >> 2) * 2 + ((lane >> 1) & 1));
    float dp[3], q[3], h[10], r[6];
    for (int k = 0; k < 3; k++) { dp[k] = in[lane * 16 + k]; q[k] = in[lane * 16 + 3 + k]; }
    for (int k = 0; k < 10; k++) h[k] = in[lane * 16 + 6 + k];
    quad_reduce_scatter(dp, q, h, quad_coef(lane, lx, ly), r, lane);
    float *dst = out + (lane >> 2) * 24 + q4;
    for (int i = 0; i < 5; i++) dst[4 * i] = r[i];
    if (q4 < 2) dst[20] = r[5];
}

constexpr int BO_PER_THREAD = 17;
__global__ void __launch_bounds__(1024)
bwd_order_kernel(ViewDev v, uint32_t *__restrict__ header, uint2 *__restrict__ bwd_items, const uint32_t *__restrict__ seg_cnt,
                 const uint32_t *__restrict__ seg_cost, const long long sst, char *__restrict__ zero_base, const long long zero_bytes,
                 const long long qst) {
    if (blockIdx.x >= 1) {
        uint4 *z = (uint4 *)l2d_view_ptr(zero_base, qst);
        const long long n16 = zero_bytes / 16;
        for (long long i = (long long)(blockIdx.x - 1) * 1024 + threadIdx.x; i < n16; i += (long long)(gridDim.x - 1) * 1024)
            z[i] = make_uint4(0u, 0u, 0u, 0u);
        return;
    }
    header = l2d_view_ptr(header, sst); bwd_items = l2d_view_ptr(bwd_items, sst); seg_cnt = l2d_view_ptr(seg_cnt, sst);
    seg_cost = l2d_view_ptr(seg_cost, sst);
    __shared__ uint32_t bcnt[64];
    if (header[1] || (v.dbg & 256u)) return;
    const int tid = threadIdx.x, lane = tid & 63;
    if (header[22]) return;
    const uint32_t n_full = header[3], n = n_full + (uint32_t)v.tiles;
    if (n > (uint32_t)(BO_PER_THREAD * 1024)) return;
    const uint32_t *cost_last = seg_cost + (v.cap / L2D_SEG + 1u);
    if (tid < 64) bcnt[tid] = 0u;
    __syncthreads();
    uint2 item[BO_PER_THREAD];
    uint32_t bkt[BO_PER_THREAD];
#pragma unroll
    for (int k = 0; k < BO_PER_THREAD; k++) {
        const uint32_t i = (uint32_t)tid + 1024u * k;
        bkt[k] = 64u;
        if (i < n) {
            uint32_t c;
            if (i < n_full) { item[k] = bwd_items[i]; c = seg_cost[i]; }
            else { const uint32_t t = i - n_full; item[k] = make_uint2(t, seg_cnt[t]); c = cost_last[t]; }
            bkt[k] = 63u - min(63u, c >> 2);
            atomicAdd(&bcnt[bkt[k]], 1u);
        }
    }
    __syncthreads();
    if (tid < 64) {
        const uint32_t c = bcnt[tid];
        uint32_t x = c;
#pragma unroll
        for (int d = 1; d < 64; d <<= 1) {
            const uint32_t y = __shfl_up(x, d, 64);
            if (lane >= d) x += y;
        }
        bcnt[tid] = x - c;
    }
    __syncthreads();
#pragma unroll
    for (int k = 0; k < BO_PER_THREAD; k++)
        if (bkt[k] < 64u) bwd_items[atomicAdd(&bcnt[bkt[k]], 1u)] = item[k];
    if (tid == 0) header[22] = 1u;
}

}

int launch_composite_fwd(const ViewDev &v, StateView st, ScratchView sc, float *out_color, float *out_allmap,
                         hipStream_t s, const ViewBatch &vb) {
    (void)sc;
    const unsigned nz = (unsigned)vb.n;
    {
        L2D_PROF(v.fwd_only ? "composite_fwd_only" : "composite_fwd", s);
        auto kern = v.fwd_only ? composite_fwd_kernel<false> : composite_fwd_kernel<true>;
        L2D_LAUNCH_IN_SCOPE(s, kern, dim3(v.tiles, 1, nz), dim3(256), 0, v, st.header, st.ranges, st.point_list,
                            (const float4 *)st.geom, st.tile_order, (const float4 *)st.cullbox, st.final_T, st.n_contrib, st.seg_base,
                            st.seg_cnt, st.ckpt, st.pair_mask, st.tile_maxc, st.seg_cost, out_color, out_allmap, vb);
    }
    return LARA2DGS_OK;
}

int launch_bwd_order(const ViewDev &v, StateView st, ScratchView sc, hipStream_t s, const ViewBatch &vb, void *zero_base, int64_t zero_bytes) {
    (void)sc;
    L2D_PROF("bwd_order", s);
    const int64_t zb = (zero_bytes + 15) / 16 * 16;
    const unsigned zw = zb > 0 ? (unsigned)((zb / 16 + 8191) / 8192 < 128 ? (zb / 16 + 8191) / 8192 : 128) : 0u;
    L2D_LAUNCH_IN_SCOPE(s, bwd_order_kernel, dim3(1 + zw, 1, (unsigned)vb.n), dim3(1024), 0, v, st.header, st.bwd_items, st.seg_cnt,
                        st.seg_cost, vb.state_stride, (char *)zero_base, (long long)zb, vb.scratch_stride);
    return LARA2DGS_OK;
}

int launch_composite_bwd(const ViewDev &v, StateView st, ScratchView sc, const float *dL_dcolor,
                         const float *dL_dallmap, hipStream_t s, const ViewBatch &vb) {
    {
        L2D_PROF(dL_dallmap ? "composite_bwd" : "composite_bwd_color", s);
        const unsigned grid = (unsigned)v.tiles + v.cap / L2D_SEG;
        auto kern = dL_dallmap ? composite_bwd_kernel<true> : composite_bwd_kernel<false>;
        L2D_LAUNCH_IN_SCOPE(s, kern, dim3(grid, 1, (unsigned)vb.n), dim3(256), 0, v, st.header, st.ranges,
                            st.point_list, (const float4 *)st.geom, st.tile_order,
                            (const float4 *)st.cullbox, st.final_T, st.n_contrib, st.seg_base, st.seg_cnt, st.bwd_order,
                            st.bwd_items, st.ckpt, st.pair_mask, st.tile_maxc, dL_dcolor, dL_dallmap, st.pair_pos, sc.pair_grad,
                            (uint8_t *)sc.pair_valid, vb);
    }
    return LARA2DGS_OK;
}

int launch_selftest_butterfly(const float *in, float *out, hipStream_t s) {
    L2D_LAUNCH_IN_SCOPE(s, selftest_butterfly_kernel, dim3(1), dim3(64), 0, in, out);
    return LARA2DGS_OK;
}
```

### lara_amd/pipeline.py

```python
from __future__ import annotations

import contextlib
import math

import os

import torch
from torch import nn

from . import _native, cameras, coarse
from .fine import _tn_over_points, fold_fine_weights, forward_fine, sample_point_feats, take_rows, take_rows_multi, voxel_rows_scenes
from .renderer import Renderer, _AssembleScenes, batch_map_buffers


class CoarseFineDecoder(nn.Module):

    def __init__(self, in_dim=80, sh_dim=12, scaling_dim=2, rotation_dim=4, opacity_dim=1, K=2):
        super().__init__()
        self.K, self.sh_dim, self.opacity_dim, self.scaling_dim, self.rotation_dim = K, sh_dim, opacity_dim, scaling_dim, rotation_dim
        self.out_dim = 3 + sh_dim + opacity_dim + scaling_dim + rotation_dim
        self.mlp_coarse = nn.Sequential(nn.Linear(in_dim, in_dim), nn.ReLU(), nn.Linear(in_dim, in_dim), nn.ReLU(),
                                        nn.Linear(in_dim, self.out_dim * K))
        self.norm = nn.LayerNorm(in_dim)
        self.cross_att = nn.MultiheadAttention(embed_dim=in_dim, num_heads=8, kdim=8, vdim=8, dropout=0.0, bias=False,
                                               batch_first=True)
        self.mlp_fine = nn.Sequential(nn.Linear(in_dim, 64), nn.ReLU(), nn.Linear(64, sh_dim))
        for seq in (self.mlp_coarse, self.mlp_fine):
            for layer in seq:
                if isinstance(layer, nn.Linear):
                    nn.init.xavier_uniform_(layer.weight)
                    nn.init.zeros_(layer.bias)


class _LinearBf16(torch.autograd.Function):

    @staticmethod
    def forward(ctx, x, weight, bias):
        xb = x.reshape(-1, x.shape[-1]).to(torch.bfloat16)
        wb = weight.to(torch.bfloat16)
        y = torch.nn.functional.linear(xb, wb, None if bias is None else bias.to(torch.bfloat16))
        ctx.save_for_backward(xb, wb)
        ctx.x_shape, ctx.x_dtype, ctx.has_bias = x.shape, x.dtype, bias is not None
        return y.view(*x.shape[:-1], weight.shape[0])

    @staticmethod
    def backward(ctx, dy):
        xb, wb = ctx.saved_tensors
        dy = dy.reshape(-1, dy.shape[-1]).to(torch.bfloat16).contiguous()
        dx = (dy @ wb).view(ctx.x_shape).to(ctx.x_dtype) if ctx.needs_input_grad[0] else None
        dw = _tn_over_points(dy, xb)
        db = dy.float().sum(0) if ctx.has_bias else None
        return dx, dw, db


def _mlp_bf16(seq, x):
    for m in seq:
        x = _LinearBf16.apply(x, m.weight, m.bias) if isinstance(m, nn.Linear) else m(x)
    return x


def decode_coarse(decoder, feats, opacity_shift, scaling_shift, autocast=True):
    par = (_mlp_bf16(decoder.mlp_coarse, feats) if autocast else decoder.mlp_coarse(feats)).float()
    K = decoder.K
    par = par.view(*par.shape[:-1], K, -1)
    offset, sh, opacity, scaling, rotation = torch.split(
        par, [3, decoder.sh_dim, decoder.opacity_dim, decoder.scaling_dim, decoder.rotation_dim], dim=-1)
    B = par.shape[0]
    return ((torch.sigmoid(offset) * 2 - 1.0).reshape(B, -1, 3), sh.reshape(B, -1, decoder.sh_dim // 3, 3),
            (scaling + scaling_shift).reshape(B, -1, decoder.scaling_dim), rotation.reshape(B, -1, decoder.rotation_dim),
            (opacity + opacity_shift).reshape(B, -1, decoder.opacity_dim))


def check_mask(mask, training, generator=None):
    m = mask.to(torch.float32)
    ratio = m.mean()
    rnd = torch.rand(mask.shape, device=mask.device, generator=generator)
    sparse = (m + rnd) > 0.8
    out = torch.where(ratio < 1e-3, sparse, mask)
    if training:
        out = torch.where(ratio > 0.5, (m * rnd) > 0.5, out)
    return out


def hand_over(obj, stream):
    if stream is None or obj is None:
        return
    if torch.is_tensor(obj):
        if obj.is_cuda:
            obj.record_stream(stream)
    elif isinstance(obj, dict):
        for v in obj.values():
            hand_over(v, stream)
    elif isinstance(obj, (list, tuple)):
        for v in obj:
            hand_over(v, stream)
    elif hasattr(obj, "__dict__"):
        for v in vars(obj).values():
            if torch.is_tensor(v):
                hand_over(v, stream)


class _TakeVoxelRows(torch.autograd.Function):

    @staticmethod
    def forward(ctx, x, vox):
        ctx.save_for_backward(vox)
        ctx.n = x.shape[0]
        return x.index_select(0, vox)

    @staticmethod
    def backward(ctx, g):
        (vox,) = ctx.saved_tensors
        out = g.new_zeros((ctx.n,) + tuple(g.shape[1:]))
        out.index_add_(0, vox, g.contiguous())
        return out, None


class LaRaPipeline(nn.Module):

    def __init__(self, vol_decoder, decoder, grid_reso=32, n_offset_groups=32, sh_degree=1, white_bkgd=True, n_views=4,
                 scene_size=0.5, n_streams=2, feat_volume=None, image_encoder=None):
        super().__init__()
        self.vol_decoder, self.decoder = vol_decoder, decoder
        self.feat_volume = feat_volume
        self.image_encoder = image_encoder
        self.K = decoder.K
        self.n_views, self.scene_size, self.n_offset_groups = n_views, scene_size, n_offset_groups
        self.gs_render = Renderer(sh_degree=sh_degree, white_background=white_bkgd, radius=1)
        self.opacity_shift = -2.1792
        self.voxel_size = 2.0 / (grid_reso * 2)
        self.scaling_shift = math.log(0.5 * self.voxel_size / 3.0)
        r = grid_reso * 2
        a = torch.arange(r)
        grid = (torch.stack(torch.meshgrid(a, a, a, indexing="ij"), dim=-1) + 0.5) / r * 2 - 1
        self.register_buffer("group_centers", (grid * scene_size).reshape(1, -1, 3).float())
        self.n_streams = n_streams
        self._streams = []
        self.fused_coarse = True
        self.fine_mask = "reference"
        self.fine_reuses_coarse_lists = True
        self.stage_events = None
        self.opacity_bias = None

    def gaussians(self, feat_vol):
        return self.gaussians_from_volume(self.vol_decoder(feat_vol))

    def gaussians_from_volume(self, vol, autocast=True):
        if autocast and self.fused_coarse and vol.is_cuda and coarse.supported(self.decoder):
            offset, shs, scaling, rotation, opacity = coarse.forward_coarse(self.decoder, vol, self.opacity_shift, self.scaling_shift)
        else:
            offset, shs, scaling, rotation, opacity = decode_coarse(self.decoder, vol, self.opacity_shift, self.scaling_shift, autocast)
        if self.opacity_bias is not None:
            opacity = opacity + self.opacity_bias
        half_cell = 0.5 * self.scene_size / self.n_offset_groups
        B = offset.shape[0]
        centers = self.group_centers.unsqueeze(-2).expand(B, -1, self.K, -1).reshape(offset.shape) + offset * half_cell
        masks = torch.sigmoid(opacity.detach()).squeeze(-1) > 0.005
        return {"centers": centers, "shs": shs, "scaling": scaling, "rotation": rotation, "opacity": opacity,
                "masks": masks, "vol": vol.view(B, -1, vol.shape[-1])}

    def trained_like_opacity_bias(self):
        r = self.group_centers.norm(dim=-1, keepdim=True)
        bias = torch.where((r - 0.35).abs() < 0.02, 4.0 - self.opacity_shift, -6.0 - self.opacity_shift)
        return bias.unsqueeze(-2).expand(-1, -1, self.K, -1).reshape(1, -1, 1).contiguous()

    @staticmethod
    def host_scalars(batch):
        packed = torch.cat([batch["near_far"].float(), batch["fovx"].float()[:, None], batch["fovy"].float()[:, None]], 1).cpu()
        return [tuple(float(x) for x in row) for row in packed]

    def scene_cameras(self, batch, i, scalars=None):
        near, far, fx, fy = (scalars or self.host_scalars(batch))[i]
        H, W = int(batch["meta"]["tar_h"][i]), int(batch["meta"]["tar_w"][i])
        return cameras.make_cameras(batch["tar_c2w"][i], W, H, fx, fy, near, far, device=batch["tar_c2w"].device)

    def _mark(self, name):
        if self.stage_events is not None:
            e = torch.cuda.Event(enable_timing=True)
            e.record()
            self.stage_events.append((name, e))

    def forward(self, batch, feat_vol, with_fine=True, n_views_sel=None, return_buffer=False):
        if n_views_sel is not None and int(n_views_sel) != self.n_views:
            raise NotImplementedError(f"lara_amd.pipeline: built for {self.n_views} input views (configs/base.yaml n_views); got n_views_sel="
                                      f"{n_views_sel} (cfg.train.use_rand_views): not supported by the fused fine stage")
        if feat_vol.dim() == 6 and feat_vol.shape[1] != self.n_views:
            raise NotImplementedError(f"lara_amd.pipeline: the image-feature volume holds {feat_vol.shape[1]} views, the pipeline is built for {self.n_views}")
        return self._step(batch, lambda: self.gaussians(feat_vol), feat_vol.device, feat_vol.shape[0], with_fine, return_buffer)

    def forward_from_image_features(self, batch, img_feats, with_fine=True, return_buffer=False):
        if self.feat_volume is None:
            raise RuntimeError("lara_amd.pipeline: forward_from_image_features needs LaRaPipeline(..., feat_volume=FeatureVolume(...))")
        from .encoder_train import VolTransformer as HipVolTransformer
        if isinstance(self.vol_decoder, HipVolTransformer):
            make = lambda: self.gaussians_from_volume(self.vol_decoder.forward_from_image_features(self.feat_volume, batch, img_feats, self.n_views))
        else:
            make = lambda: self.gaussians(self.feat_volume(batch, img_feats, self.n_views))
        return self._step(batch, make, img_feats.device, batch["tar_rays_down"].shape[0], with_fine, return_buffer)

    def forward_from_images(self, batch, with_fine=True, return_buffer=False):
        if self.image_encoder is None:
            raise RuntimeError("lara_amd.pipeline: forward_from_images needs LaRaPipeline(..., image_encoder=DinoViT(...))")
        if self.feat_volume is None:
            raise RuntimeError("lara_amd.pipeline: forward_from_images needs LaRaPipeline(..., feat_volume=FeatureVolume(...))")
        return self.forward_from_image_features(batch, self.image_encoder.image_features(batch, self.n_views), with_fine, return_buffer)

    def forward_from_volume(self, batch, volume_feat_up, with_fine=True, autocast=True, return_buffer=False):
        return self._step(batch, lambda: self.gaussians_from_volume(volume_feat_up, autocast), volume_feat_up.device,
                          volume_feat_up.shape[0], with_fine, return_buffer)

    def _step(self, batch, make_gaussians, dev, B, with_fine, return_buffer=False):
        _native.require_device(dev)
        n_sel = self.n_views
        scalars = self.host_scalars(batch)
        cur = torch.cuda.current_stream(dev)
        n_streams = min(self.n_streams, B)
        while len(self._streams) < n_streams and n_streams > 1:
            self._streams.append(torch.cuda.Stream(dev))
        sides = self._streams[:n_streams] if n_streams > 1 else [None] * B
        on = lambda s: torch.cuda.stream(s) if s is not None else contextlib.nullcontext()

        sizes = [(int(batch["meta"]["tar_w"][i]), int(batch["meta"]["tar_h"][i])) for i in range(B)]
        cams_of = cameras.make_cameras_scenes(batch["tar_c2w"], sizes, scalars, device=batch["tar_c2w"].device)
        bg_rows = torch.nn.functional.pad(batch["bg_color"].float(), (0, 1))[..., :3]
        self._mark("start")
        g = make_gaussians()
        inps = batch["tar_rgb"][:, :n_sel].permute(0, 1, 4, 2, 3).float().contiguous()
        if with_fine:
            masks = g["masks"]
            if self.fine_mask == "reference":
                masks = torch.stack([check_mask(masks[i], self.training) for i in range(B)])
        self._mark("encoder+decoder")
        bufs = None
        if len(set(sizes)) == 1 and len({len(c) for c in cams_of}) == 1:
            bufs = batch_map_buffers(B, sizes[0][1], sizes[0][0] * len(cams_of[0]), dev, ("", "_fine") if with_fine else ("",))
        for s in sides:
            if s is not None:
                s.wait_stream(cur)
                hand_over((g, inps, cams_of, bufs, bg_rows, [batch[k] for k in ("tar_rays", "bg_color", "tar_w2c", "tar_ixt") if k in batch]), s)

        sc = {k: g[k].unbind(0) for k in ("centers", "shs", "opacity", "scaling", "rotation")}
        per_scene = [None] * B
        buffers = [[(sc["centers"][i], sc["shs"][i], sc["opacity"][i], sc["scaling"][i], sc["rotation"][i])] for i in range(B)] \
            if return_buffer else None
        coarse_raster = [[] for _ in range(B)]
        for i in range(B):
            s = sides[i % len(sides)]
            with on(s):
                per_scene[i] = self.gs_render.render_views(
                    cams_of[i], batch["tar_rays"][i], sc["centers"][i], sc["shs"][i], sc["opacity"][i], sc["scaling"][i],
                    sc["rotation"][i], dev, bg_colors=bg_rows[i], concat=True,
                    into=None if bufs is None else {k: v[i] for k, v in bufs.items() if not k.endswith("_fine")},
                    raster_out=coarse_raster[i])
                self._mark("coarse views")
        if with_fine:
            idx = [masks[i].nonzero().squeeze(-1) for i in range(B)]
            folded = fold_fine_weights(self.decoder)
            vox = [torch.div(idx[i], self.K, rounding_mode="floor") for i in range(B)]
            vol_rows = voxel_rows_scenes(g["vol"], vox)
            for s in sides:
                if s is not None:
                    s.wait_stream(cur)
                    hand_over((masks, folded, vol_rows), s)
            for i in range(B):
                s = sides[i % len(sides)]
                hand_over(idx[i], s)
                with on(s):
                    co = per_scene[i]
                    H, VW = co["acc_map"].shape
                    V, W = len(cams_of[i]), VW // len(cams_of[i])
                    five = [sc["centers"][i], sc["shs"][i], sc["opacity"][i], sc["scaling"][i], sc["rotation"][i]]
                    centers_f, shs_sel, opacity_f, scaling_f, rotation_f = take_rows_multi(five, idx[i])
                    pf = sample_point_feats(centers_f, batch["tar_w2c"][i, :n_sel], batch["tar_ixt"][i, :n_sel], inps[i],
                                            co["image"], co["acc_map"], co["depth"], row_views=V)
                    sh_res = forward_fine(self.decoder, vol_rows[i], torch.einsum("lcb->blc", pf), folded)
                    shs_f = sh_res.view(-1, *g["shs"].shape[-2:]) + shs_sel
                    if return_buffer:
                        buffers[i].append((centers_f, shs_f, sc["opacity"][i], sc["scaling"][i], sc["rotation"][i], masks[i]))
                    self._mark("sampler+forward_fine")
                    co.update(self.gs_render.render_views(
                        cams_of[i], batch["tar_rays"][i], centers_f, shs_f, opacity_f, scaling_f, rotation_f, dev,
                        bg_colors=bg_rows[i], prex="_fine", concat=True,
                        into=None if bufs is None else {k: v[i] for k, v in bufs.items() if k.endswith("_fine")},
                        subset_of=(coarse_raster[i][0][0], idx[i]) if self.fine_reuses_coarse_lists else None))
                    self._mark("fine views")
        outs = per_scene
        for i, s in enumerate(sides):
            if s is not None:
                cur.wait_stream(s)
        if sides[0] is not None:
            hand_over(per_scene, cur)
            if buffers is not None:
                hand_over(buffers, cur)
        if bufs is not None:
            out = {k: _AssembleScenes.apply(bufs[k], *[o[k] for o in outs]) for k in outs[0]}
        else:
            out = {k: torch.stack([o[k] for o in outs]) for k in outs[0]}
        if return_buffer:
            out["render_pkg"] = [t for scene in buffers for t in scene]
        self._mark("outputs")
        return out

    def join_streams(self):
        cur = torch.cuda.current_stream()
        for s in self._streams:
            cur.wait_stream(s)


def lara_loss(batch, output, it=10000, ms_ssim=True):
    from .loss import ms_ssim_terms
    B, V, H, W = batch["tar_rgb"].shape[:-1]
    tar = batch["tar_rgb"].permute(0, 2, 1, 3, 4).reshape(B, H, V * W, 3)
    loss, stats = 0, {}
    for prex in ("", "_fine"):
        if f"image{prex}" not in output:
            continue
        if prex == "_fine" and "acc_map_fine" not in output:
            continue
        mse = ((output[f"image{prex}"] - tar) ** 2).mean()
        loss = loss + mse
        stats[f"mse{prex}"] = mse.detach()
        stats[f"psnr{prex}"] = -10.0 * torch.log10(mse.detach())
        if ms_ssim:
            extra, st = ms_ssim_terms(batch, output, (prex,), fused=False)
            loss = loss + extra[prex]
            stats.update(st)
        if f"rend_dist{prex}" in output and it > 1000 and prex != "_fine":
            dist = output[f"rend_dist{prex}"].mean()
            err = ((1 - (output[f"rend_normal{prex}"] * output[f"depth_normal{prex}"]).sum(dim=-1))
                   * output[f"acc_map{prex}"].detach()).mean()
            loss = loss + dist * 1000 + err * 0.2
            stats[f"distortion{prex}"], stats[f"normal{prex}"] = dist.detach(), err.detach()
    return loss, stats
```

### lara_amd/rasterizer.py

```python
from __future__ import annotations

import collections
import os
import threading
import time
import warnings
from typing import NamedTuple, Optional

import torch
from torch import nn

from . import _native
from ._native import (ABI_VERSION, LIB_PATH, GradLayout, StateLayout, Subset as _Subset, View as _View,
                      alloc_bytes as _alloc_bytes, check as _check, check_poison_guards, _poison_mode)


def load_library():
    return _native.load_library(LIB_PATH)


_cull_transparent = os.environ.get("LARA2DGS_CULL_TRANSPARENT", "0") == "1"


_TIGHT_TILES_BIT = 4


def _flag_bits(rs, tight_tiles: bool) -> int:
    return int(bool(rs.prefiltered)) | (2 if _cull_transparent else 0) | (_TIGHT_TILES_BIT if tight_tiles else 0)


def set_cull_transparent(on: bool) -> bool:
    global _cull_transparent
    prev, _cull_transparent = _cull_transparent, bool(on)
    return prev


def _dup_factor() -> int:
    return int(os.environ.get("LARA2DGS_DUP_FACTOR", "4"))


def _sizing_P(P: int) -> int:
    if P <= 32768:
        return max(-(-P // 1024) * 1024, 1024)
    return (P + 32767) // 65536 * 65536 + 32768


_HISTORY = 256
_hist = {}
_reruns = 0


def _bucket(device: torch.device, P: int, H: int, W: int, tight_tiles: bool = False):
    b = (device.index, _sizing_P(P), int(H), int(W))
    return b + ("tight_tiles",) if tight_tiles else b


def _cap_grid(n: int) -> int:
    n = max(int(n), 1 << 20)
    k = 1 << (n - 1).bit_length()
    if k // 4 * 3 >= n:
        k = k // 4 * 3
    return min(k, 0xFFFFFFFF)


def note_pair_count(bucket, D: int):
    h = _hist.get(bucket)
    if h is None:
        h = _hist[bucket] = collections.deque(maxlen=_HISTORY)
    h.append(int(D))


def _recent_max(bucket) -> int:
    h = _hist.get(bucket)
    return max(h) if h else 0


def _next_capacity(bucket) -> int:
    return _cap_grid(max(bucket[1] * _dup_factor(), 2 * _recent_max(bucket)))


def binning_capacity(P: int, H: int = 0, W: int = 0, device: Optional[torch.device] = None) -> int:
    if device is None:
        return _cap_grid(_sizing_P(P) * _dup_factor())
    return _next_capacity(_bucket(device, P, H, W))


_longest = {}


def capacity_report() -> dict:
    rep = {b: {"D_max": max(h), "calls": len(h), "capacity": _cap_grid(max(b[1] * _dup_factor(), 2 * max(h))),
               "longest_list": _longest.get(b, 0)}
           for b, h in _hist.items() if h}
    rep["reruns"] = _reruns
    return rep


def reset_capacity_history():
    _hist.clear()
    _longest.clear()


_tls = threading.local()
_COUNT_SPINS = 4000
_counts_fallbacks = 0


class _Counts:

    def __init__(self, n):
        self.t = torch.zeros((max(n, 16), 4), dtype=torch.int32).pin_memory()
        self.np = self.t.numpy().view("uint32")
        self.ptr = self.t.data_ptr()


def _counts(n) -> _Counts:
    c = getattr(_tls, "counts", None)
    if c is None or c.np.shape[0] < n:
        c = _tls.counts = _Counts(n)
    return c


def _wait_counts(c: _Counts, n: int, done: torch.cuda.Event, headers):
    global _counts_fallbacks
    ready = c.np[:n, 3]
    spins = 0
    while not ready.all():
        spins += 1
        if spins > _COUNT_SPINS:
            if done.query() and not ready.all():
                _counts_fallbacks += 1
                h = headers().cpu().numpy().view("uint32").reshape(n, -1)
                return int(h[:, 0].max()), bool(h[:, 1].any())
            time.sleep(0)
    return int(c.np[:n, 0].max()), bool(c.np[:n, 1].any())


def _run_forward(bucket, n, enqueue, debug=False):
    global _reruns
    cap = _next_capacity(bucket)
    c = _counts(n)
    while True:
        c.np[:n, 3] = 0
        state, headers, extra = enqueue(cap, c.ptr)
        done = torch.cuda.Event()
        done.record()
        D, overflow = _wait_counts(c, n, done, headers)
        note_pair_count(bucket, D)
        if bool(c.np[:n, 3].all()):
            _longest[bucket] = max(_longest.get(bucket, 0), int(c.np[:n, 2].max()))
        if not overflow:
            break
        new_cap = _cap_grid(max(2 * D, bucket[1] * _dup_factor()))
        if new_cap <= cap:
            raise RuntimeError(
                f"lara_amd: a view produced {D} (tile, surfel) pairs, beyond the 32-bit pair index the buffers use "
                f"(capacity {cap}); its outputs were poisoned with NaN.")
        _reruns += 1
        state = headers = None
        cap = new_cap
    if debug:
        torch.cuda.current_stream().synchronize()
    return state, cap, extra, D


_scratch = {}


def _get_scratch(device: torch.device, nbytes: int) -> torch.Tensor:
    if _poison_mode():
        return _alloc_bytes(nbytes, device)
    key = (device.index, _native.current_stream(device))
    buf = _scratch.get(key)
    if buf is None or buf.numel() < nbytes:
        buf = torch.empty(int(nbytes * 1.25) + 256, dtype=torch.uint8, device=device)
        _scratch[key] = buf
    return buf


def _prep(t: Optional[torch.Tensor], name: str, device) -> Optional[torch.Tensor]:
    if t is None or t.numel() == 0:
        return None
    if t.device != device:
        raise RuntimeError(f"lara_amd: `{name}` is on {t.device}, expected {device}")
    if t.dtype != torch.float32:
        if not t.is_floating_point():
            raise RuntimeError(f"lara_amd: `{name}` must be a floating-point tensor, got {t.dtype}")
        t = t.float()
    if not t.is_contiguous():
        t = t.contiguous()
    if t.data_ptr() % 16:
        t = t.clone()
    return t


class GaussianRasterizationSettings(NamedTuple):
    image_height: int
    image_width: int
    tanfovx: float
    tanfovy: float
    bg: torch.Tensor
    scale_modifier: float
    viewmatrix: torch.Tensor
    projmatrix: torch.Tensor
    sh_degree: int
    campos: torch.Tensor
    prefiltered: bool
    debug: bool


def _make_view(rs: GaussianRasterizationSettings, P: int, M: int, cap: int, device, tight_tiles=False):
    bg = _prep(rs.bg, "bg", device)
    vm = _prep(rs.viewmatrix, "viewmatrix", device)
    pm = _prep(rs.projmatrix, "projmatrix", device)
    cp = _prep(rs.campos, "campos", device)
    if bg is None or vm is None or pm is None or cp is None:
        raise RuntimeError("lara_amd: bg / viewmatrix / projmatrix / campos must be non-empty tensors")
    if bg.numel() != 3 or vm.numel() != 16 or pm.numel() != 16 or cp.numel() != 3:
        raise RuntimeError("lara_amd: bg[3], viewmatrix[4,4], projmatrix[4,4], campos[3] expected")
    v = _View(P, int(rs.sh_degree), M, int(rs.image_height), int(rs.image_width),
              float(rs.tanfovx), float(rs.tanfovy), float(rs.scale_modifier),
              _flag_bits(rs, tight_tiles), int(bool(rs.debug)), 0, cap,
              bg.data_ptr(), vm.data_ptr(), pm.data_ptr(), cp.data_ptr(), None)
    return v, (bg, vm, pm, cp)


def _validate(means3D, sh, colors_precomp, opacities, scales, rotations, cov3Ds_precomp, sh_degree):
    if means3D.dim() != 2 or means3D.shape[1] != 3:
        raise RuntimeError("means3D must have dimensions (num_points, 3)")
    _native.require_device(means3D)
    device = means3D.device
    P = means3D.shape[0]
    means3D_c = _prep(means3D, "means3D", device)
    if means3D_c is None:
        means3D_c = means3D.contiguous()
    sh_c = _prep(sh, "shs", device)
    col_c = _prep(colors_precomp, "colors_precomp", device)
    opa_c = _prep(opacities, "opacities", device)
    sc_c = _prep(scales, "scales", device)
    rot_c = _prep(rotations, "rotations", device)
    tm_c = _prep(cov3Ds_precomp, "cov3D_precomp", device)
    M = 0
    if sh_c is not None:
        if sh_c.dim() != 3 or sh_c.shape[0] != P or sh_c.shape[2] != 3:
            raise RuntimeError("shs must have dimensions (num_points, num_coeffs, 3)")
        M = sh_c.shape[1]
        if M < (int(sh_degree) + 1) ** 2:
            raise RuntimeError("shs holds fewer coefficients than sh_degree needs")
    for t, n, k in ((opa_c, "opacities", 1), (sc_c, "scales", 2), (rot_c, "rotations", 4),
                    (tm_c, "cov3D_precomp", 9), (col_c, "colors_precomp", 3)):
        if t is not None and t.numel() != P * k:
            raise RuntimeError(f"{n} must hold {k} value(s) per point")
    return device, P, M, (means3D_c, sh_c, col_c, opa_c, sc_c, rot_c, tm_c)


def _needs_state(*tensors) -> bool:
    return torch.is_grad_enabled() and any(t is not None and t.requires_grad for t in tensors)


def _views_array(settings, P, M, cap, device, tight_tiles=False):
    arr = (_View * len(settings))()
    keep = []
    for i, rs in enumerate(settings):
        v, k = _make_view(rs, P, M, cap, device, tight_tiles)
        arr[i] = v
        keep.extend(k)
    return arr, keep


def _forward_views_impl(means3D, sh, colors_precomp, opacities, scales, rotations, cov3Ds_precomp, settings, forward_only=False,
                        subset=None, batched=True, tight_tiles=False):
    lib = load_library()
    rs0 = settings[0]
    n = len(settings)
    for rs in settings[1:]:
        if (rs.image_height, rs.image_width, rs.sh_degree, bool(rs.prefiltered), float(rs.scale_modifier), bool(rs.debug)) != \
                (rs0.image_height, rs0.image_width, rs0.sh_degree, bool(rs0.prefiltered), float(rs0.scale_modifier), bool(rs0.debug)):
            raise RuntimeError("lara_amd: the views of one multi-view call must agree in image size, sh_degree, prefiltered, "
                               "scale_modifier and debug")
    device, P, M, (means3D_c, sh_c, col_c, opa_c, sc_c, rot_c, tm_c) = _validate(
        means3D, sh, colors_precomp, opacities, scales, rotations, cov3Ds_precomp, rs0.sh_degree)
    H, W = int(rs0.image_height), int(rs0.image_width)
    fo = int(bool(forward_only))
    with torch.cuda.device(device):
        views, keep = _views_array(settings, P, M, 0, device, tight_tiles)
        lead = (n,) if batched else ()
        color = torch.empty(lead + (3, H, W), dtype=torch.float32, device=device)
        allmap = torch.empty(lead + (7, H, W), dtype=torch.float32, device=device)
        radii = torch.empty(lead + (P,), dtype=torch.int32, device=device)
        sub = None
        if subset is not None and P > 0:
            c_state, c_sb, c_cap, c_P, idx = subset
            if idx.numel() != P or idx.device != device or c_P < P:
                raise RuntimeError("lara_amd: `subset_of` needs one index per surfel of this call, on its device")
            inv = torch.full((c_P,), -1, dtype=torch.int32, device=device)
            inv[idx] = torch.arange(P, dtype=torch.int32, device=device)
            sub = _Subset(c_state.data_ptr(), c_sb, c_cap, c_P, 0, inv.data_ptr())

        def enqueue(cap, counts_ptr):
            for i in range(n):
                views[i].capacity = cap
                views[i].forward_only = fo
                views[i].counts_out = counts_ptr + 16 * i
            sb = (lib.lara2dgs_state_bytes(_sizing_P(P), H, W, cap, fo) + 255) // 256 * 256
            qb = (lib.lara2dgs_scratch_bytes(_sizing_P(P), H, W, cap, fo) + 255) // 256 * 256
            state = _alloc_bytes(n * sb, device)
            scratch = _get_scratch(device, n * qb)
            args = (n, views, *_native.pointers(means3D_c, sh_c, col_c, opa_c, sc_c, rot_c, tm_c, color, allmap, radii, state),
                    sb, scratch.data_ptr(), qb)
            if sub is None:
                _check(lib.lara2dgs_forward_views(*args, _native.current_stream(device)), "lara2dgs_forward_views")
            else:
                _check(lib.lara2dgs_forward_views_subset(*args, sub, _native.current_stream(device)),
                       "lara2dgs_forward_views_subset")
            return state, (lambda: state.view(n, sb)[:, :64].contiguous().view(torch.int32)), (sb, qb)

        state, cap, (sb, qb), D = _run_forward(_bucket(device, P, H, W, tight_tiles), n, enqueue, any(rs.debug for rs in settings))
    return dict(color=color, radii=radii, allmap=allmap, state=state, cap=cap, strides=(sb, qb), D=D, M=M, keep=keep,
                prefiltered_bits=int(views[0].prefiltered), inputs=(means3D_c, sh_c, col_c, sc_c, rot_c, tm_c))


class _RasterizeViews(torch.autograd.Function):

    @staticmethod
    def forward(ctx, means3D, means2D, sh, colors_precomp, opacities, scales, rotations, cov3Ds_precomp, settings, subset=None,
                batched=True, tight_tiles=False):
        settings = tuple(settings)
        r = _forward_views_impl(means3D, sh, colors_precomp, opacities, scales, rotations, cov3Ds_precomp, settings, subset=subset,
                                batched=batched, tight_tiles=tight_tiles)
        color, radii, allmap, M, keep = r["color"], r["radii"], r["allmap"], r["M"], r["keep"]
        means3D_c, sh_c, col_c, sc_c, rot_c, tm_c = r["inputs"]
        ctx.state, ctx.cap, ctx.strides, ctx.D = r["state"], r["cap"], r["strides"], r["D"]
        ctx.settings = settings
        ctx.M = M
        ctx.prefiltered_bits = r["prefiltered_bits"]
        ctx.flags = (sh_c is not None, col_c is not None, sc_c is not None, tm_c is not None)
        ctx.shapes = (sh.shape if sh_c is not None else None, opacities.shape)
        empty = means3D_c.new_empty(0)
        ctx.save_for_backward(means3D_c, sh_c if sh_c is not None else empty, col_c if col_c is not None else empty,
                              sc_c if sc_c is not None else empty, rot_c if rot_c is not None else empty,
                              tm_c if tm_c is not None else empty, radii, *keep)
        ctx.mark_non_differentiable(radii)
        ctx.set_materialize_grads(False)
        return color, radii, allmap

    @staticmethod
    def backward(ctx, grad_color, grad_radii, grad_allmap):
        lib = load_library()
        means3D, sh, col, sc, rot, tm, radii = ctx.saved_tensors[:7]
        cams = ctx.saved_tensors[7:]
        has_sh, has_col, has_sr, has_tm = ctx.flags
        settings = ctx.settings
        n = len(settings)
        rs0 = settings[0]
        device = means3D.device
        P = means3D.shape[0]
        H, W = int(rs0.image_height), int(rs0.image_width)
        state, cap, (sb, qb) = ctx.state, ctx.cap, ctx.strides
        G = GradLayout()
        _check(lib.lara2dgs_get_grad_layout(P, ctx.M, int(has_sh), int(has_col), int(has_sr), int(has_tm), G),
               "lara2dgs_get_grad_layout")
        with torch.cuda.device(device):
            if grad_color is None:
                grad_color = torch.zeros((n, 3, H, W), dtype=torch.float32, device=device)
            grad_color = _prep(grad_color, "grad_color", device)
            if grad_allmap is not None:
                grad_allmap = _prep(grad_allmap, "grad_allmap", device)
            views = (_View * n)()
            for i, rs in enumerate(settings):
                bg, vm, pm, cp = cams[4 * i:4 * i + 4]
                views[i] = _View(P, int(rs.sh_degree), ctx.M, H, W, float(rs.tanfovx), float(rs.tanfovy),
                                 float(rs.scale_modifier), ctx.prefiltered_bits, int(bool(rs.debug)), 0, cap,
                                 bg.data_ptr(), vm.data_ptr(), pm.data_ptr(), cp.data_ptr(), None)
            out = torch.empty((max(G.total, 4),), dtype=torch.float32, device=device)
            scratch = _get_scratch(device, n * qb)
            ptrs = _native.pointers(means3D, sh if has_sh else None, col if has_col else None, sc if has_sr else None,
                                    rot if has_sr else None, tm if has_tm else None, radii, grad_color, grad_allmap, state)
            _check(lib.lara2dgs_backward_views(n, views, *ptrs, sb, scratch.data_ptr(), qb, out.data_ptr(),
                                               _native.current_stream(device)), "lara2dgs_backward_views")

        def sec(off, k, shape):
            return None if off < 0 else out[off:off + P * k].view(shape)
        g_sh = sec(G.shs, ctx.M * 3, (P, ctx.M, 3)) if has_sh else None
        if g_sh is not None and ctx.shapes[0] is not None:
            g_sh = g_sh.view(ctx.shapes[0])
        g_opac = sec(G.opacities, 1, (P, 1)).view(ctx.shapes[1])
        return (sec(G.means3D, 3, (P, 3)), sec(G.means2D, 3, (P, 3)) if ctx.needs_input_grad[1] else None, g_sh,
                sec(G.colors, 3, (P, 3)) if has_col else None, g_opac,
                sec(G.scales, 2, (P, 2)) if has_sr else None, sec(G.rotations, 4, (P, 4)) if has_sr else None,
                sec(G.transmat, 9, (P, 9)) if has_tm else None, None, None, None, None)


def rasterize_gaussians_views(settings, means3D, means2D, opacities, shs=None, colors_precomp=None, scales=None,
                              rotations=None, cov3D_precomp=None, subset_of=None, tight_tiles=False):
    if len(settings) == 0:
        raise RuntimeError("lara_amd: rasterize_gaussians_views needs at least one view")
    if (shs is None and colors_precomp is None) or (shs is not None and colors_precomp is not None):
        raise Exception('Please provide excatly one of either SHs or precomputed colors!')
    if ((scales is None or rotations is None) and cov3D_precomp is None) or \
            ((scales is not None or rotations is not None) and cov3D_precomp is not None):
        raise Exception('Please provide exactly one of either scale/rotation pair or precomputed 3D covariance!')
    means3D, means2D, shs, colors_precomp, opacities, scales, rotations, cov3D_precomp = (
        _as_f32(t) for t in (means3D, means2D, shs, colors_precomp, opacities, scales, rotations, cov3D_precomp))
    if not _needs_state(means3D, means2D, shs, colors_precomp, opacities, scales, rotations, cov3D_precomp):
        r = _forward_views_impl(means3D, shs, colors_precomp, opacities, scales, rotations, cov3D_precomp, tuple(settings), True,
                                tight_tiles=tight_tiles)
        return r["color"], r["radii"], r["allmap"]
    subset = None
    if subset_of is not None:
        coarse_color, idx = subset_of
        node = getattr(coarse_color, "grad_fn", None)
        if node is not None and hasattr(node, "strides") and hasattr(node, "state") and len(node.settings) == len(settings):
            for a, b in zip(node.settings, settings):
                if (a.image_height, a.image_width, a.tanfovx, a.tanfovy, float(a.scale_modifier)) != \
                        (b.image_height, b.image_width, b.tanfovx, b.tanfovy, float(b.scale_modifier)) or \
                        a.viewmatrix.data_ptr() != b.viewmatrix.data_ptr() or a.projmatrix.data_ptr() != b.projmatrix.data_ptr():
                    raise RuntimeError("lara_amd: `subset_of` names a call with other cameras")
            if node.prefiltered_bits != _flag_bits(settings[0], tight_tiles):
                raise RuntimeError("lara_amd: `subset_of` names a call made with other flags (prefiltered / cull_transparent / "
                                   f"tight_tiles bits {node.prefiltered_bits}, this call's {_flag_bits(settings[0], tight_tiles)}): "
                                   "its lists were binned under another rule than this call's counts")
            subset = (node.state, node.strides[0], node.cap, node.saved_tensors[0].shape[0], idx.contiguous())
    return _RasterizeViews.apply(means3D, means2D, shs, colors_precomp, opacities, scales, rotations, cov3D_precomp,
                                 tuple(settings), subset, True, bool(tight_tiles))


def _as_f32(t):
    return t.float() if (t is not None and t.is_floating_point() and t.dtype != torch.float32) else t


def rasterize_gaussians(means3D, means2D, sh, colors_precomp, opacities, scales, rotations,
                        cov3Ds_precomp, raster_settings, tight_tiles=False):
    means3D, means2D, sh, colors_precomp, opacities, scales, rotations, cov3Ds_precomp = (
        _as_f32(t) for t in (means3D, means2D, sh, colors_precomp, opacities, scales, rotations, cov3Ds_precomp))
    if not _needs_state(means3D, means2D, sh, colors_precomp, opacities, scales, rotations, cov3Ds_precomp):
        r = _forward_views_impl(means3D, sh, colors_precomp, opacities, scales, rotations, cov3Ds_precomp, (raster_settings,), True,
                                batched=False, tight_tiles=tight_tiles)
        return r["color"], r["radii"], r["allmap"]
    return _RasterizeViews.apply(means3D, means2D, sh, colors_precomp, opacities, scales, rotations, cov3Ds_precomp,
                                 (raster_settings,), None, False, bool(tight_tiles))


class GaussianRasterizer(nn.Module):

    def __init__(self, raster_settings: GaussianRasterizationSettings):
        super().__init__()
        self.raster_settings = raster_settings

    def markVisible(self, positions: torch.Tensor) -> torch.Tensor:
        rs = self.raster_settings
        with torch.no_grad():
            if not positions.is_cuda:
                raise RuntimeError("lara_amd: tensors must live on an MI355X (HIP) device")
            device = positions.device
            pos = _prep(positions, "positions", device)
            P = positions.shape[0]
            present = torch.zeros((P,), dtype=torch.uint8, device=device)
            vm = _prep(rs.viewmatrix, "viewmatrix", device)
            pm = _prep(rs.projmatrix, "projmatrix", device)
            _native.call("lara2dgs_mark_visible", device, P, pos, vm, pm, present)
        return present.bool()

    def forward(self, means3D, means2D, opacities, shs=None, colors_precomp=None, scales=None,
                rotations=None, cov3D_precomp=None):
        raster_settings = self.raster_settings
        if (shs is None and colors_precomp is None) or (shs is not None and colors_precomp is not None):
            raise Exception('Please provide excatly one of either SHs or precomputed colors!')
        if ((scales is None or rotations is None) and cov3D_precomp is None) or \
                ((scales is not None or rotations is not None) and cov3D_precomp is not None):
            raise Exception('Please provide exactly one of either scale/rotation pair or precomputed 3D covariance!')
        return rasterize_gaussians(means3D, means2D, shs, colors_precomp, opacities, scales,
                                   rotations, cov3D_precomp, raster_settings)


def state_views(state: torch.Tensor, P: int, H: int, W: int, cap: int, forward_only: bool = False) -> dict:
    L = StateLayout()
    _native.call("lara2dgs_get_state_layout", None, P, H, W, cap, int(forward_only), L)
    tiles = ((W + 15) // 16) * ((H + 15) // 16)

    def sec(off, nbytes, dtype, shape):
        return state[off:off + nbytes].view(dtype).view(shape)

    hdr = sec(L.header, 256, torch.int32, (64,))
    common = dict(
        header=hdr,
        geom=sec(L.geom, P * 80, torch.float32, (P, 20)),
        cullbox=sec(L.cullbox, P * 16, torch.float32, (P, 4)),
        point_list=sec(L.point_list, cap * 4, torch.int32, (cap,)),
        ranges=sec(L.ranges, tiles * 8, torch.int32, (tiles, 2)),
        tile_order=sec(L.tile_order, tiles * 4, torch.int32, (tiles,)))
    if forward_only:
        return common
    return dict(
        common,
        pair_base=sec(L.pair_base, (P + 1) * 4, torch.int32, (P + 1,)),
        pair_pos=sec(L.pair_pos, cap * 4, torch.int32, (cap,)),
        final_T=sec(L.final_T, 10 * H * W * 4, torch.float32, (10, H, W)),
        n_contrib=sec(L.n_contrib, 2 * H * W * 4, torch.int32, (2, H, W)),
        seg_base=sec(L.seg_base, (tiles + 1) * 4, torch.int32, (tiles + 1,)),
        seg_cnt=sec(L.seg_cnt, tiles * 4, torch.int32, (tiles,)),
        bwd_order=sec(L.bwd_order, tiles * 4, torch.int32, (tiles,)),
        bwd_items=sec(L.bwd_items, (cap // 512 + 1 + tiles) * 8, torch.int32, (cap // 512 + 1 + tiles, 2)),
        pair_mask=sec(L.pair_mask, cap * 8, torch.int64, (cap,)),
        tile_maxc=sec(L.tile_maxc, tiles * 4, torch.int32, (tiles,)),
        seg_cost=sec(L.seg_cost, (cap // 512 + 1 + tiles) * 4, torch.int32, (cap // 512 + 1 + tiles,)),
    )


def forward_with_state(raster_settings, means3D, opacities, shs=None, colors_precomp=None,
                       scales=None, rotations=None, cov3D_precomp=None, forward_only=False, tight_tiles=False) -> dict:
    with torch.no_grad():
        r = _forward_views_impl(means3D, shs, colors_precomp, opacities, scales, rotations, cov3D_precomp, (raster_settings,),
                                forward_only, batched=False, tight_tiles=tight_tiles)
    P = means3D.shape[0]
    r["views"] = state_views(r["state"], P, int(raster_settings.image_height),
                             int(raster_settings.image_width), r["cap"], forward_only)
    return r


def profile_enable(on: bool = True):
    load_library().lara2dgs_profile_enable(int(on))


def profile_collect(max_entries: int = 65536) -> list:
    names = _native.char_buffer(max_entries * 24)
    ms = _native.host_array("f", max_entries)
    n = load_library().lara2dgs_profile_collect(names, len(names), ms, max_entries)
    parts = names.raw.split(b"\0")
    return [(parts[i].decode(), float(ms[i])) for i in range(n)]
```

### lara_amd/renderer.py

```python
from __future__ import annotations

import math
import os

import torch
from torch import nn

from ._native import call, require_device
from .rasterizer import GaussianRasterizationSettings, GaussianRasterizer, rasterize_gaussians, rasterize_gaussians_views


class _SurfaceMaps(torch.autograd.Function):

    @staticmethod
    def forward(ctx, color, allmap, rays, rot, depth_ratio):
        require_device(color)
        color, allmap = color.float().contiguous(), allmap.float().contiguous()
        rays, rot = rays.detach().float().contiguous(), rot.detach().float().contiguous()
        H, W = color.shape[1], color.shape[2]
        if allmap.shape != (7, H, W) or rays.shape != (H, W, 6) or rot.shape != (3, 3):
            raise RuntimeError("expected color [3,H,W], allmap [7,H,W], rays [H,W,6], rot [3,3]")
        o = dict(dtype=torch.float32, device=color.device)
        image, depth, acc = torch.empty(H, W, 3, **o), torch.empty(H, W, 1, **o), torch.empty(H, W, **o)
        rnorm, dnorm, rdist = torch.empty(H, W, 3, **o), torch.empty(H, W, 3, **o), torch.empty(H, W, **o)
        call("lara_surface_maps_forward", color.device, H, W, color, allmap, rays, rot, float(depth_ratio), image, depth, acc, rnorm,
             dnorm, rdist)
        ctx.save_for_backward(color, allmap, rays, rot)
        ctx.depth_ratio = float(depth_ratio)
        ctx.set_materialize_grads(False)
        return image, depth, acc, rnorm, dnorm, rdist

    @staticmethod
    def backward(ctx, g_image, g_depth, g_acc, g_rnorm, g_dnorm, g_rdist):
        color, allmap, rays, rot = ctx.saved_tensors
        H, W = color.shape[1], color.shape[2]
        gs = [None if g is None else g.float().contiguous() for g in (g_image, g_depth, g_acc, g_rnorm, g_dnorm, g_rdist)]
        d_color = torch.empty_like(color)
        d_allmap = None if all(g is None for g in gs[1:]) else torch.empty_like(allmap)
        call("lara_surface_maps_backward", color.device, H, W, color, allmap, rays, rot, ctx.depth_ratio, *gs, d_color, d_allmap)
        return d_color, d_allmap, None, None, None


class _Activate(torch.autograd.Function):

    @staticmethod
    def forward(ctx, opacity, scales, rotations):
        require_device(opacity)
        P = opacity.shape[0]
        if opacity.shape != (P, 1) or scales.shape != (P, 2) or rotations.shape != (P, 4):
            raise RuntimeError("expected opacity [P,1], scales [P,2], rotations [P,4]")
        o, s, r = (t.detach().float().contiguous() for t in (opacity, scales, rotations))
        oa, sa, ra = torch.empty_like(o), torch.empty_like(s), torch.empty_like(r)
        call("lara_activate_gaussians_forward", o.device, P, o, s, r, oa, sa, ra)
        ctx.save_for_backward(oa, sa, r)
        ctx.set_materialize_grads(False)
        return oa, sa, ra

    @staticmethod
    def backward(ctx, g_o, g_s, g_r):
        oa, sa, r = ctx.saved_tensors
        P = oa.shape[0]
        gs = [None if g is None else g.float().contiguous() for g in (g_o, g_s, g_r)]
        need = ctx.needs_input_grad
        d = [torch.empty_like(t) if n else None for t, n in zip((oa, sa, r), need)]
        call("lara_activate_gaussians_backward", oa.device, P, oa, sa, r, *gs, *d)
        return tuple(d)


def activate_gaussians(opacity, scales, rotations):
    return _Activate.apply(opacity, scales, rotations)


class _SurfaceMapsViews(torch.autograd.Function):

    @staticmethod
    def forward(ctx, color, allmap, rays, rots, depth_ratio, into=None):
        require_device(color)
        color, allmap = color.float().contiguous(), allmap.float().contiguous()
        rays, rots = rays.detach().float().contiguous(), rots.detach().float().contiguous()
        n, H, W = color.shape[0], color.shape[2], color.shape[3]
        if color.shape != (n, 3, H, W) or allmap.shape != (n, 7, H, W) or rays.shape != (n, H, W, 6) or rots.shape != (n, 3, 3):
            raise RuntimeError("expected color [n,3,H,W], allmap [n,7,H,W], rays [n,H,W,6], rots [n,3,3]")
        o = dict(dtype=torch.float32, device=color.device)
        shapes = ((H, n * W, 3), (H, n * W, 1), (H, n * W), (H, n * W, 3), (H, n * W, 3), (H, n * W))
        if into is None:
            image, depth, acc, rnorm, dnorm, rdist = (torch.empty(*sh, **o) for sh in shapes)
        else:
            for t, sh in zip(into, shapes):
                if tuple(t.shape) != sh or t.dtype != torch.float32 or not t.is_contiguous() or t.device != color.device or t.requires_grad:
                    raise RuntimeError("lara_amd: `into` buffers must be contiguous fp32 tensors of the maps' shapes that need no gradient")
            image, depth, acc, rnorm, dnorm, rdist = (t.detach() for t in into)
        call("lara_surface_maps_forward_views", color.device, n, H, W, color, allmap, rays, rots, float(depth_ratio), image, depth,
             acc, rnorm, dnorm, rdist)
        ctx.save_for_backward(color, allmap, rays, rots)
        ctx.depth_ratio = float(depth_ratio)
        ctx.set_materialize_grads(False)
        return image, depth, acc, rnorm, dnorm, rdist

    @staticmethod
    def backward(ctx, g_image, g_depth, g_acc, g_rnorm, g_dnorm, g_rdist):
        color, allmap, rays, rots = ctx.saved_tensors
        n, H, W = color.shape[0], color.shape[2], color.shape[3]
        gs = [None if g is None else g.float().contiguous() for g in (g_image, g_depth, g_acc, g_rnorm, g_dnorm, g_rdist)]
        d_color = torch.empty_like(color)
        d_allmap = None if all(g is None for g in gs[1:]) else torch.empty_like(allmap)
        call("lara_surface_maps_backward_views", color.device, n, H, W, color, allmap, rays, rots, ctx.depth_ratio, *gs, d_color,
             d_allmap)
        return d_color, d_allmap, None, None, None, None


def surface_maps_views(color, allmap, rays, rots, depth_ratio=0.0, into=None):
    return _SurfaceMapsViews.apply(color, allmap, rays, rots, depth_ratio, into)


MAP_KEYS = ("image", "depth", "acc_map", "rend_normal", "depth_normal", "rend_dist")


class _AssembleScenes(torch.autograd.Function):

    @staticmethod
    def forward(ctx, buf, *parts):
        for i, p in enumerate(parts):
            if p.data_ptr() != buf[i].data_ptr() or p.shape != buf[i].shape:
                raise RuntimeError("lara_amd: a scene's map does not live in its slice of the batch buffer")
        return buf.detach()

    @staticmethod
    def backward(ctx, g):
        return (None,) + tuple(g.unbind(0))


def batch_map_buffers(B, H, VW, device, prexes=("",)):
    o = dict(dtype=torch.float32, device=device)
    chans = {"image": (3,), "depth": (1,), "acc_map": (), "rend_normal": (3,), "depth_normal": (3,), "rend_dist": ()}
    return {k + prex: torch.empty((B, H, VW) + chans[k], **o) for prex in prexes for k in MAP_KEYS}


def surface_maps(color, allmap, rays, rot, depth_ratio=0.0):
    return _SurfaceMaps.apply(color, allmap, rays, rot, depth_ratio)


class Renderer(nn.Module):

    def __init__(self, sh_degree=3, white_background=True, radius=1, tight_tiles=None):
        super().__init__()
        self.tight_tiles = (os.environ.get("LARA2DGS_TIGHT_TILES", "1") == "1") if tight_tiles is None else bool(tight_tiles)
        self.sh_degree, self.white_background, self.radius = sh_degree, white_background, radius
        self.scaling_activation, self.opacity_activation = torch.exp, torch.sigmoid
        self.rotation_activation = torch.nn.functional.normalize
        self.bg_color = torch.tensor([1, 1, 1] if white_background else [0, 0, 0], dtype=torch.float32)
        self._act_key, self._act_val = None, None

    def set_bg_color(self, bg):
        self.bg_color = bg

    def _settings(self, viewpoint_camera, scaling_modifier=1.0, device="cuda", bg=None):
        return GaussianRasterizationSettings(
            image_height=int(viewpoint_camera.image_height), image_width=int(viewpoint_camera.image_width),
            tanfovx=math.tan(viewpoint_camera.FoVx * 0.5), tanfovy=math.tan(viewpoint_camera.FoVy * 0.5),
            bg=(self.bg_color if bg is None else bg).to(device), scale_modifier=scaling_modifier,
            viewmatrix=viewpoint_camera.world_view_transform, projmatrix=viewpoint_camera.full_proj_transform,
            sh_degree=self.sh_degree, campos=viewpoint_camera.camera_center, prefiltered=False, debug=False)

    def set_rasterizer(self, viewpoint_camera, scaling_modifier=1.0, device="cuda"):
        return GaussianRasterizer(raster_settings=self._settings(viewpoint_camera, scaling_modifier, device))

    def get_opacity(self, _opacity):
        return self.opacity_activation(_opacity)

    def get_scaling(self, _scaling):
        return self.scaling_activation(_scaling)

    def get_rotation(self, _rotation):
        return self.rotation_activation(_rotation)

    def _zero_means2D(self, centers):
        z = getattr(self, "_zeros2d", None)
        if z is None or z.shape != centers.shape or z.device != centers.device or z.dtype != centers.dtype:
            z = torch.zeros_like(centers, requires_grad=False)
            self._zeros2d = z
        return z

    @staticmethod
    def _tensor_key(t):
        if t is None:
            return None
        base = t._base if t._is_view() else t
        return (id(base), t.data_ptr(), t.storage_offset(), tuple(t.shape), tuple(t.stride()), t.dtype, t.device,
                t._version, t.requires_grad)

    def _activated(self, opacity, scales, rotations):
        key = tuple(self._tensor_key(t) for t in (opacity, scales, rotations)) + (torch.is_grad_enabled(),)
        if key != self._act_key:
            fused = (scales is not None and rotations is not None and opacity.is_cuda and opacity.dim() == 2
                     and self.scaling_activation is torch.exp and self.opacity_activation is torch.sigmoid
                     and self.rotation_activation is torch.nn.functional.normalize)
            if fused:
                self._act_val = activate_gaussians(opacity, scales, rotations) + ((opacity, scales, rotations),)
            else:
                self._act_val = (self.get_opacity(opacity), None if scales is None else self.get_scaling(scales),
                                 None if rotations is None else self.get_rotation(rotations), (opacity, scales, rotations))
            self._act_key = key
        return self._act_val[:3]

    def invalidate_activations(self):
        self._act_key, self._act_val = None, None

    def render_img(self, cam, rays, centers, shs, opacity, scales, rotations, device, cov3D_precomp=None, prex='',
                   depth_ratio=0.0):
        settings = self._settings(cam, device=device)
        opacity, scales, rotations = self._activated(opacity, scales, rotations)
        screenspace_points = self._zero_means2D(centers)
        rendered_image, radii, allmap = rasterize_gaussians(centers, screenspace_points, shs, None, opacity, scales, rotations,
                                                            cov3D_precomp, settings, tight_tiles=self.tight_tiles)
        if rays is None:
            return rendered_image.clamp(0, 1)
        rot = cam.world_view_transform[:3, :3].T
        image, depth, acc, rnorm, dnorm, rdist = surface_maps(rendered_image, allmap, rays, rot, depth_ratio)
        return {f"image{prex}": image, f"depth{prex}": depth, f"acc_map{prex}": acc, f"rend_normal{prex}": rnorm,
                f"depth_normal{prex}": dnorm, f"rend_dist{prex}": rdist}

    def render_views(self, cams, rays, centers, shs, opacity, scales, rotations, device, bg_colors=None,
                     cov3D_precomp=None, prex='', depth_ratio=0.0, concat=False, into=None, raster_out=None, subset_of=None):
        n = len(cams)
        if torch.is_tensor(bg_colors) and bg_colors.dim() == 2 and not (
                bg_colors.dtype == torch.float32 and bg_colors.stride() == (4, 1) and bg_colors.data_ptr() % 16 == 0):
            bg_colors = torch.nn.functional.pad(bg_colors.float(), (0, 1))[:, :3]
        bgs = [None] * n if bg_colors is None else list(bg_colors)
        settings = [self._settings(cam, device=device, bg=bg) for cam, bg in zip(cams, bgs)]
        opacity, scales, rotations = self._activated(opacity, scales, rotations)
        color, radii, allmap = rasterize_gaussians_views(settings, centers, self._zero_means2D(centers), opacity, shs=shs,
                                                         scales=scales, rotations=rotations, cov3D_precomp=cov3D_precomp,
                                                         subset_of=subset_of, tight_tiles=self.tight_tiles)
        if raster_out is not None:
            raster_out.append((color, radii, allmap))
        if concat and rays is not None:
            rots = torch.stack([cam.world_view_transform[:3, :3] for cam in cams]).transpose(1, 2)
            rays_t = rays if torch.is_tensor(rays) else torch.stack(list(rays))
            image, depth, acc, rnorm, dnorm, rdist = surface_maps_views(
                color, allmap, rays_t, rots, depth_ratio, None if into is None else tuple(into[k + prex] for k in MAP_KEYS))
            return {f"image{prex}": image, f"depth{prex}": depth, f"acc_map{prex}": acc, f"rend_normal{prex}": rnorm,
                    f"depth_normal{prex}": dnorm, f"rend_dist{prex}": rdist}
        out = []
        for i, cam in enumerate(cams):
            if rays is None:
                out.append(color[i].clamp(0, 1))
                continue
            rot = cam.world_view_transform[:3, :3].T
            image, depth, acc, rnorm, dnorm, rdist = surface_maps(color[i], allmap[i], rays[i], rot, depth_ratio)
            out.append({f"image{prex}": image, f"depth{prex}": depth, f"acc_map{prex}": acc, f"rend_normal{prex}": rnorm,
                        f"depth_normal{prex}": dnorm, f"rend_dist{prex}": rdist})
        return out
```

Measured before the change: 945.5.

## Skip median-depth tracking when unused and add 4-WG colour-only backward variant

Adds a no-median template path to the forward and backward composite kernels. It is enabled by default when depth_ratio is 0 and the allmap does not escape to the caller, and it drops the per-pixel median depth/contributor tracking, its store, and its gradient term. It also adds a colour-only backward variant with a smaller LDS pool and launch bounds that allow four workgroups per CU, chosen by a work-item threshold. The pipeline now passes only the colour tensor instead of the full raster tuple, so the skip path can apply there. The risk is that median depth becomes 0 in the allmap, which is only correct if nothing downstream reads it. The smaller pool may also cause more slab refills.

```diff
diff --git a/lara_amd/csrc/abi.hip b/lara_amd/csrc/abi.hip
--- a/lara_amd/csrc/abi.hip
+++ b/lara_amd/csrc/abi.hip
@@ -59,6 +59,8 @@
     v.scale_modifier = view->scale_modifier;
     v.cull_transparent = (view->prefiltered >> 1) & 1;
     v.tight_tiles = (view->prefiltered >> 2) & 1;
+    v.no_median = (view->prefiltered >> 3) & 1;
+    v.color_bwd_wg4 = (view->prefiltered >> 4) & 1;
     v.cap = (unsigned)view->capacity;
     v.fwd_only = view->forward_only != 0;
     v.counts_out = view->counts_out;
diff --git a/lara_amd/csrc/common.h b/lara_amd/csrc/common.h
--- a/lara_amd/csrc/common.h
+++ b/lara_amd/csrc/common.h
@@ -26,6 +26,8 @@
     unsigned dbg;
     int cull_transparent;
     int tight_tiles;
+    int no_median;
+    int color_bwd_wg4;
     int fwd_only;
     const float *bg, *viewmatrix, *projmatrix, *campos;
     uint32_t *counts_out;
diff --git a/lara_amd/csrc/composite.hip b/lara_amd/csrc/composite.hip
--- a/lara_amd/csrc/composite.hip
+++ b/lara_amd/csrc/composite.hip
@@ -171,7 +171,7 @@
     uint32_t last_contributor = 0, median_contributor = 0;
     bool done = false;
 
-    template <int CHUNK>
+    template <int CHUNK, bool MED>
     __device__ __forceinline__ void blend(const float4 *rec, const int j, const int base, bool valid,
                                           const Hit &h) {
         valid = valid && !done;
@@ -190,9 +190,11 @@
         Dd += depth * w;
         M1 += mm * w;
         M2 += mm * mm * w;
-        const bool med = valid && T > 0.5f;
-        median_depth = med ? depth : median_depth;
-        median_contributor = med ? (uint32_t)(base + j + 1) : median_contributor;
+        if constexpr (MED) {
+            const bool med = valid && T > 0.5f;
+            median_depth = med ? depth : median_depth;
+            median_contributor = med ? (uint32_t)(base + j + 1) : median_contributor;
+        }
         N0 += r4.x * w; N1 += r4.y * w; N2 += r4.z * w;
         C0 += r4.w * w; C1 += r5.x * w; C2 += r5.y * w;
         T = valid ? test_T : T;
@@ -201,7 +203,7 @@
 
 };
 
-template <bool KEEP>
+template <bool KEEP, bool MED>
 __global__ void __launch_bounds__(256)
 composite_fwd_kernel(ViewDev v, const uint32_t *__restrict__ header, const uint2 *__restrict__ ranges,
                      const uint32_t *__restrict__ point_list, const float4 *__restrict__ geom,
@@ -248,7 +250,8 @@
             for (int ch = 0; ch < 7; ch++) out_allmap[ch * HW + pix] = qnan;
             if (KEEP) {
                 for (int ch = 0; ch < L2D_CKPT_F; ch++) final_T[pix + ch * HW] = qnan;
-                n_contrib[pix] = 0; n_contrib[pix + HW] = 0;
+                n_contrib[pix] = 0;
+                if (MED) n_contrib[pix + HW] = 0;
             }
         }
         return;
@@ -354,8 +357,8 @@
                 atomicAdd(&dbg_hdr[5], (unsigned)e0 + (unsigned)e1);
                 if (lane == 0) atomicAdd(&dbg_hdr[6], 1u);
             }
-            px.blend<CHUNK>(rec, j0, base, e0, h0);
-            px.blend<CHUNK>(rec, j1, base, e1, h1);
+            px.blend<CHUNK, MED>(rec, j0, base, e0, h0);
+            px.blend<CHUNK, MED>(rec, j1, base, e1, h1);
             if (((__ballot(px.done) >> (lane & ~3)) & 0xfull) == 0xfull) { mm = 0ull; w = nw; n0 = false; n1 = false; }
         };
         uint32_t ntrips = 0;
@@ -392,7 +395,7 @@
             final_T[pix + 6 * HW] = px.Dd;
             final_T[pix + 7 * HW] = px.N0; final_T[pix + 8 * HW] = px.N1; final_T[pix + 9 * HW] = px.N2;
             n_contrib[pix] = px.last_contributor;
-            n_contrib[pix + HW] = px.median_contributor;
+            if (MED) n_contrib[pix + HW] = px.median_contributor;
         }
         out_color[0 * HW + pix] = px.C0 + T * v.bg[0];
         out_color[1 * HW + pix] = px.C1 + T * v.bg[1];
@@ -402,7 +405,7 @@
         out_allmap[2 * HW + pix] = px.N0;
         out_allmap[3 * HW + pix] = px.N1;
         out_allmap[4 * HW + pix] = px.N2;
-        out_allmap[5 * HW + pix] = px.median_depth;
+        out_allmap[5 * HW + pix] = MED ? px.median_depth : 0.0f;
         out_allmap[6 * HW + pix] = px.distortion;
         if ((v.dbg & 32u) && lane == 0) {
             out_allmap[6 * HW + pix] = (float)((long long)__builtin_readcyclecounter() - dbg_t0);
@@ -489,9 +492,10 @@
 constexpr int SLAB_F = 24;
 constexpr int SLAB_F_COLOR = 16;
 constexpr int SLAB_POOL_COLOR = SLAB_POOL * SLAB_F / SLAB_F_COLOR;
-
-template <bool MAPS>
-__global__ void __launch_bounds__(256)
+constexpr int SLAB_POOL_COLOR4 = 370;
+
+template <bool MAPS, bool MED, bool WG4>
+__global__ void __launch_bounds__(256, WG4 ? 4 : 1)
 composite_bwd_kernel(ViewDev v, const uint32_t *__restrict__ header, const uint2 *__restrict__ ranges,
                      const uint32_t *__restrict__ point_list, const float4 *__restrict__ geom,
                      const uint32_t *__restrict__ tile_order, const float4 *__restrict__ cullbox,
@@ -516,7 +520,8 @@
         v.bg = vb.bg[blockIdx.z];
     }
     constexpr int WIN = SLAB_WIN;
-    constexpr int POOL = MAPS ? SLAB_POOL : SLAB_POOL_COLOR, SF = MAPS ? SLAB_F : SLAB_F_COLOR;
+    static_assert(!(MAPS && WG4), "only the colour-only form is built for four workgroups per CU");
+    constexpr int POOL = MAPS ? SLAB_POOL : (WG4 ? SLAB_POOL_COLOR4 : SLAB_POOL_COLOR), SF = MAPS ? SLAB_F : SLAB_F_COLOR;
     __shared__ float4 rec[REC4 * WIN];
     __shared__ __attribute__((aligned(16))) float pool[(POOL + 1) * SF];
     __shared__ uint16_t s_base_[2][SLAB_CHUNK];
@@ -570,7 +575,7 @@
     const float T_final = inside ? final_T[pix] : 0.f;
     float T = T_final;
     const uint32_t last_contributor = inside ? n_contrib[pix] : 0u;
-    const uint32_t median_contributor = (MAPS && inside) ? n_contrib[pix + HW] : 0u;
+    const uint32_t median_contributor = (MAPS && MED && inside) ? n_contrib[pix + HW] : 0u;
     float dpix[3] = {0.f, 0.f, 0.f}, dnrm[3] = {0.f, 0.f, 0.f};
     float dL_ddepth = 0.f, dL_daccum = 0.f, dL_dmedian = 0.f, dL_dreg = 0.f;
     float final_D = 0.f, final_D2 = 0.f;
@@ -580,7 +585,7 @@
             dL_ddepth = dL_dallmap[0 * HW + pix];
             dL_daccum = dL_dallmap[1 * HW + pix];
             for (int ch = 0; ch < 3; ch++) dnrm[ch] = dL_dallmap[(2 + ch) * HW + pix];
-            dL_dmedian = dL_dallmap[5 * HW + pix];
+            if constexpr (MED) dL_dmedian = dL_dallmap[5 * HW + pix];
             dL_dreg = dL_dallmap[6 * HW + pix];
             final_D = final_T[pix + HW];
             final_D2 = final_T[pix + 2 * HW];
@@ -591,6 +596,8 @@
 
     float accum_g = 0.f, last_g = 0.f, last_alpha = 0.f;
     float last_dL_dT = 0.f;
+    float dz_zero = 0.0f;
+    if constexpr (MAPS && !MED) asm volatile("" : "+v"(dz_zero));
 
     const int my_blk = (lyi >> 1) * 8 + (lxi >> 1);
     const uint32_t below_lo = my_blk >= 32 ? 0xffffffffu : (1u << my_blk) - 1u;
@@ -795,11 +802,11 @@
                                        c_d * dL_ddepth + dL_daccum;
                     const float accum_new = mul_legacy(last_alpha, last_g) + (1.f - last_alpha) * accum_g;
                     float dL_dalpha = gval - accum_new;
-                    float dL_dz = 0.0f;
+                    float dL_dz = (MAPS && !MED) ? dz_zero : 0.0f;
                     const float inv_cd = __builtin_amdgcn_rcpf(c_d);
                     const float m_d = FAR_N / (FAR_N - NEAR_N) * (1.f - NEAR_N * inv_cd);
                     const float dmd_dd = (FAR_N * NEAR_N) / (FAR_N - NEAR_N) * inv_cd * inv_cd;
-                    if (contributor + 1 == median_contributor) dL_dz += dL_dmedian;
+                    if constexpr (MED) { if (contributor + 1 == median_contributor) dL_dz += dL_dmedian; }
                     const float dL_dweight = (final_D2 + m_d * m_d * final_A - 2.f * m_d * final_D) * dL_dreg;
                     dL_dalpha += dL_dweight - last_dL_dT;
                     const float dLdT_new = mul_legacy(alpha, dL_dweight) + (1.f - alpha) * last_dL_dT;
@@ -1044,7 +1051,8 @@
     const unsigned nz = (unsigned)vb.n;
     {
         L2D_PROF(v.fwd_only ? "composite_fwd_only" : "composite_fwd", s);
-        auto kern = v.fwd_only ? composite_fwd_kernel<false> : composite_fwd_kernel<true>;
+        auto kern = v.no_median ? (v.fwd_only ? composite_fwd_kernel<false, false> : composite_fwd_kernel<true, false>)
+                                : (v.fwd_only ? composite_fwd_kernel<false, true> : composite_fwd_kernel<true, true>);
         L2D_LAUNCH_IN_SCOPE(s, kern, dim3(v.tiles, 1, nz), dim3(256), 0, v, st.header, st.ranges, st.point_list,
                             (const float4 *)st.geom, st.tile_order, (const float4 *)st.cullbox, st.final_T, st.n_contrib, st.seg_base,
                             st.seg_cnt, st.ckpt, st.pair_mask, st.tile_maxc, st.seg_cost, out_color, out_allmap, vb);
@@ -1067,7 +1075,8 @@
     {
         L2D_PROF(dL_dallmap ? "composite_bwd" : "composite_bwd_color", s);
         const unsigned grid = (unsigned)v.tiles + v.cap / L2D_SEG;
-        auto kern = dL_dallmap ? composite_bwd_kernel<true> : composite_bwd_kernel<false>;
+        auto kern = dL_dallmap ? (v.no_median ? composite_bwd_kernel<true, false, false> : composite_bwd_kernel<true, true, false>)
+                               : (v.color_bwd_wg4 ? composite_bwd_kernel<false, true, true> : composite_bwd_kernel<false, true, false>);
         L2D_LAUNCH_IN_SCOPE(s, kern, dim3(grid, 1, (unsigned)vb.n), dim3(256), 0, v, st.header, st.ranges,
                             st.point_list, (const float4 *)st.geom, st.tile_order,
                             (const float4 *)st.cullbox, st.final_T, st.n_contrib, st.seg_base, st.seg_cnt, st.bwd_order,
diff --git a/lara_amd/pipeline.py b/lara_amd/pipeline.py
--- a/lara_amd/pipeline.py
+++ b/lara_amd/pipeline.py
@@ -243,7 +243,7 @@
         per_scene = [None] * B
         buffers = [[(sc["centers"][i], sc["shs"][i], sc["opacity"][i], sc["scaling"][i], sc["rotation"][i])] for i in range(B)] \
             if return_buffer else None
-        coarse_raster = [[] for _ in range(B)]
+        coarse_color = [[] for _ in range(B)]
         for i in range(B):
             s = sides[i % len(sides)]
             with on(s):
@@ -251,7 +251,7 @@
                     cams_of[i], batch["tar_rays"][i], sc["centers"][i], sc["shs"][i], sc["opacity"][i], sc["scaling"][i],
                     sc["rotation"][i], dev, bg_colors=bg_rows[i], concat=True,
                     into=None if bufs is None else {k: v[i] for k, v in bufs.items() if not k.endswith("_fine")},
-                    raster_out=coarse_raster[i])
+                    color_out=coarse_color[i])
                 self._mark("coarse views")
         if with_fine:
             idx = [masks[i].nonzero().squeeze(-1) for i in range(B)]
@@ -282,7 +282,7 @@
                         cams_of[i], batch["tar_rays"][i], centers_f, shs_f, opacity_f, scaling_f, rotation_f, dev,
                         bg_colors=bg_rows[i], prex="_fine", concat=True,
                         into=None if bufs is None else {k: v[i] for k, v in bufs.items() if k.endswith("_fine")},
-                        subset_of=(coarse_raster[i][0][0], idx[i]) if self.fine_reuses_coarse_lists else None))
+                        subset_of=(coarse_color[i][0], idx[i]) if self.fine_reuses_coarse_lists else None))
                     self._mark("fine views")
         outs = per_scene
         for i, s in enumerate(sides):
diff --git a/lara_amd/rasterizer.py b/lara_amd/rasterizer.py
--- a/lara_amd/rasterizer.py
+++ b/lara_amd/rasterizer.py
@@ -23,10 +23,24 @@
 
 
 _TIGHT_TILES_BIT = 4
-
-
-def _flag_bits(rs, tight_tiles: bool) -> int:
-    return int(bool(rs.prefiltered)) | (2 if _cull_transparent else 0) | (_TIGHT_TILES_BIT if tight_tiles else 0)
+_NO_MEDIAN_BIT = 8
+_COLOR_BWD_WG4_BIT = 16
+_BINNING_BITS = ~_NO_MEDIAN_BIT
+
+COLOR_BWD_WG4_MIN_WORK_ITEMS = 1536
+_SEGMENT = 512
+_color_bwd_force = None
+
+
+def color_bwd_four_workgroups(pairs: int, n_views: int, tiles: int) -> bool:
+    if _color_bwd_force is not None:
+        return int(_color_bwd_force) == 4
+    return n_views * tiles + pairs // _SEGMENT >= COLOR_BWD_WG4_MIN_WORK_ITEMS
+
+
+def _flag_bits(rs, tight_tiles: bool, no_median: bool = False) -> int:
+    return int(bool(rs.prefiltered)) | (2 if _cull_transparent else 0) | (_TIGHT_TILES_BIT if tight_tiles else 0) | \
+        (_NO_MEDIAN_BIT if no_median else 0)
 
 
 def set_cull_transparent(on: bool) -> bool:
@@ -159,6 +173,7 @@
         _reruns += 1
         state = headers = None
         cap = new_cap
+    _tls.pairs_in_all = int(c.np[:n, 0].sum()) if bool(c.np[:n, 3].all()) else n * D
     if debug:
         torch.cuda.current_stream().synchronize()
     return state, cap, extra, D
@@ -209,7 +224,7 @@
     debug: bool
 
 
-def _make_view(rs: GaussianRasterizationSettings, P: int, M: int, cap: int, device, tight_tiles=False):
+def _make_view(rs: GaussianRasterizationSettings, P: int, M: int, cap: int, device, tight_tiles=False, no_median=False):
     bg = _prep(rs.bg, "bg", device)
     vm = _prep(rs.viewmatrix, "viewmatrix", device)
     pm = _prep(rs.projmatrix, "projmatrix", device)
@@ -220,7 +235,7 @@
         raise RuntimeError("lara_amd: bg[3], viewmatrix[4,4], projmatrix[4,4], campos[3] expected")
     v = _View(P, int(rs.sh_degree), M, int(rs.image_height), int(rs.image_width),
               float(rs.tanfovx), float(rs.tanfovy), float(rs.scale_modifier),
-              _flag_bits(rs, tight_tiles), int(bool(rs.debug)), 0, cap,
+              _flag_bits(rs, tight_tiles, no_median), int(bool(rs.debug)), 0, cap,
               bg.data_ptr(), vm.data_ptr(), pm.data_ptr(), cp.data_ptr(), None)
     return v, (bg, vm, pm, cp)
 
@@ -258,18 +273,18 @@
     return torch.is_grad_enabled() and any(t is not None and t.requires_grad for t in tensors)
 
 
-def _views_array(settings, P, M, cap, device, tight_tiles=False):
+def _views_array(settings, P, M, cap, device, tight_tiles=False, no_median=False):
     arr = (_View * len(settings))()
     keep = []
     for i, rs in enumerate(settings):
-        v, k = _make_view(rs, P, M, cap, device, tight_tiles)
+        v, k = _make_view(rs, P, M, cap, device, tight_tiles, no_median)
         arr[i] = v
         keep.extend(k)
     return arr, keep
 
 
 def _forward_views_impl(means3D, sh, colors_precomp, opacities, scales, rotations, cov3Ds_precomp, settings, forward_only=False,
-                        subset=None, batched=True, tight_tiles=False):
+                        subset=None, batched=True, tight_tiles=False, no_median=False):
     lib = load_library()
     rs0 = settings[0]
     n = len(settings)
@@ -283,7 +298,7 @@
     H, W = int(rs0.image_height), int(rs0.image_width)
     fo = int(bool(forward_only))
     with torch.cuda.device(device):
-        views, keep = _views_array(settings, P, M, 0, device, tight_tiles)
+        views, keep = _views_array(settings, P, M, 0, device, tight_tiles, no_median)
         lead = (n,) if batched else ()
         color = torch.empty(lead + (3, H, W), dtype=torch.float32, device=device)
         allmap = torch.empty(lead + (7, H, W), dtype=torch.float32, device=device)
@@ -316,7 +331,8 @@
             return state, (lambda: state.view(n, sb)[:, :64].contiguous().view(torch.int32)), (sb, qb)
 
         state, cap, (sb, qb), D = _run_forward(_bucket(device, P, H, W, tight_tiles), n, enqueue, any(rs.debug for rs in settings))
-    return dict(color=color, radii=radii, allmap=allmap, state=state, cap=cap, strides=(sb, qb), D=D, M=M, keep=keep,
+        D_sum = _tls.pairs_in_all
+    return dict(color=color, radii=radii, allmap=allmap, state=state, cap=cap, strides=(sb, qb), D=D, D_sum=D_sum, M=M, keep=keep,
                 prefiltered_bits=int(views[0].prefiltered), inputs=(means3D_c, sh_c, col_c, sc_c, rot_c, tm_c))
 
 
@@ -324,13 +340,13 @@
 
     @staticmethod
     def forward(ctx, means3D, means2D, sh, colors_precomp, opacities, scales, rotations, cov3Ds_precomp, settings, subset=None,
-                batched=True, tight_tiles=False):
+                batched=True, tight_tiles=False, no_median=False):
         settings = tuple(settings)
         r = _forward_views_impl(means3D, sh, colors_precomp, opacities, scales, rotations, cov3Ds_precomp, settings, subset=subset,
-                                batched=batched, tight_tiles=tight_tiles)
+                                batched=batched, tight_tiles=tight_tiles, no_median=no_median)
         color, radii, allmap, M, keep = r["color"], r["radii"], r["allmap"], r["M"], r["keep"]
         means3D_c, sh_c, col_c, sc_c, rot_c, tm_c = r["inputs"]
-        ctx.state, ctx.cap, ctx.strides, ctx.D = r["state"], r["cap"], r["strides"], r["D"]
+        ctx.state, ctx.cap, ctx.strides, ctx.D, ctx.D_sum = r["state"], r["cap"], r["strides"], r["D"], r["D_sum"]
         ctx.settings = settings
         ctx.M = M
         ctx.prefiltered_bits = r["prefiltered_bits"]
@@ -367,10 +383,13 @@
             if grad_allmap is not None:
                 grad_allmap = _prep(grad_allmap, "grad_allmap", device)
             views = (_View * n)()
+            bits = ctx.prefiltered_bits
+            if grad_allmap is None and color_bwd_four_workgroups(ctx.D_sum, n, ((W + 15) // 16) * ((H + 15) // 16)):
+                bits |= _COLOR_BWD_WG4_BIT
             for i, rs in enumerate(settings):
                 bg, vm, pm, cp = cams[4 * i:4 * i + 4]
                 views[i] = _View(P, int(rs.sh_degree), ctx.M, H, W, float(rs.tanfovx), float(rs.tanfovy),
-                                 float(rs.scale_modifier), ctx.prefiltered_bits, int(bool(rs.debug)), 0, cap,
+                                 float(rs.scale_modifier), bits, int(bool(rs.debug)), 0, cap,
                                  bg.data_ptr(), vm.data_ptr(), pm.data_ptr(), cp.data_ptr(), None)
             out = torch.empty((max(G.total, 4),), dtype=torch.float32, device=device)
             scratch = _get_scratch(device, n * qb)
@@ -388,11 +407,11 @@
         return (sec(G.means3D, 3, (P, 3)), sec(G.means2D, 3, (P, 3)) if ctx.needs_input_grad[1] else None, g_sh,
                 sec(G.colors, 3, (P, 3)) if has_col else None, g_opac,
                 sec(G.scales, 2, (P, 2)) if has_sr else None, sec(G.rotations, 4, (P, 4)) if has_sr else None,
-                sec(G.transmat, 9, (P, 9)) if has_tm else None, None, None, None, None)
+                sec(G.transmat, 9, (P, 9)) if has_tm else None, None, None, None, None, None)
 
 
 def rasterize_gaussians_views(settings, means3D, means2D, opacities, shs=None, colors_precomp=None, scales=None,
-                              rotations=None, cov3D_precomp=None, subset_of=None, tight_tiles=False):
+                              rotations=None, cov3D_precomp=None, subset_of=None, tight_tiles=False, _no_median=False):
     if len(settings) == 0:
         raise RuntimeError("lara_amd: rasterize_gaussians_views needs at least one view")
     if (shs is None and colors_precomp is None) or (shs is not None and colors_precomp is not None):
@@ -404,7 +423,7 @@
         _as_f32(t) for t in (means3D, means2D, shs, colors_precomp, opacities, scales, rotations, cov3D_precomp))
     if not _needs_state(means3D, means2D, shs, colors_precomp, opacities, scales, rotations, cov3D_precomp):
         r = _forward_views_impl(means3D, shs, colors_precomp, opacities, scales, rotations, cov3D_precomp, tuple(settings), True,
-                                tight_tiles=tight_tiles)
+                                tight_tiles=tight_tiles, no_median=_no_median)
         return r["color"], r["radii"], r["allmap"]
     subset = None
     if subset_of is not None:
@@ -416,13 +435,13 @@
                         (b.image_height, b.image_width, b.tanfovx, b.tanfovy, float(b.scale_modifier)) or \
                         a.viewmatrix.data_ptr() != b.viewmatrix.data_ptr() or a.projmatrix.data_ptr() != b.projmatrix.data_ptr():
                     raise RuntimeError("lara_amd: `subset_of` names a call with other cameras")
-            if node.prefiltered_bits != _flag_bits(settings[0], tight_tiles):
+            if (node.prefiltered_bits & _BINNING_BITS) != _flag_bits(settings[0], tight_tiles):
                 raise RuntimeError("lara_amd: `subset_of` names a call made with other flags (prefiltered / cull_transparent / "
-                                   f"tight_tiles bits {node.prefiltered_bits}, this call's {_flag_bits(settings[0], tight_tiles)}): "
+                                   f"tight_tiles bits {node.prefiltered_bits & _BINNING_BITS}, this call's {_flag_bits(settings[0], tight_tiles)}): "
                                    "its lists were binned under another rule than this call's counts")
             subset = (node.state, node.strides[0], node.cap, node.saved_tensors[0].shape[0], idx.contiguous())
     return _RasterizeViews.apply(means3D, means2D, shs, colors_precomp, opacities, scales, rotations, cov3D_precomp,
-                                 tuple(settings), subset, True, bool(tight_tiles))
+                                 tuple(settings), subset, True, bool(tight_tiles), bool(_no_median))
 
 
 def _as_f32(t):
@@ -430,15 +449,15 @@
 
 
 def rasterize_gaussians(means3D, means2D, sh, colors_precomp, opacities, scales, rotations,
-                        cov3Ds_precomp, raster_settings, tight_tiles=False):
+                        cov3Ds_precomp, raster_settings, tight_tiles=False, _no_median=False):
     means3D, means2D, sh, colors_precomp, opacities, scales, rotations, cov3Ds_precomp = (
         _as_f32(t) for t in (means3D, means2D, sh, colors_precomp, opacities, scales, rotations, cov3Ds_precomp))
     if not _needs_state(means3D, means2D, sh, colors_precomp, opacities, scales, rotations, cov3Ds_precomp):
         r = _forward_views_impl(means3D, sh, colors_precomp, opacities, scales, rotations, cov3Ds_precomp, (raster_settings,), True,
-                                batched=False, tight_tiles=tight_tiles)
+                                batched=False, tight_tiles=tight_tiles, no_median=_no_median)
         return r["color"], r["radii"], r["allmap"]
     return _RasterizeViews.apply(means3D, means2D, sh, colors_precomp, opacities, scales, rotations, cov3Ds_precomp,
-                                 (raster_settings,), None, False, bool(tight_tiles))
+                                 (raster_settings,), None, False, bool(tight_tiles), bool(_no_median))
 
 
 class GaussianRasterizer(nn.Module):
@@ -508,10 +527,11 @@
 
 
 def forward_with_state(raster_settings, means3D, opacities, shs=None, colors_precomp=None,
-                       scales=None, rotations=None, cov3D_precomp=None, forward_only=False, tight_tiles=False) -> dict:
+                       scales=None, rotations=None, cov3D_precomp=None, forward_only=False, tight_tiles=False,
+                       _no_median=False) -> dict:
     with torch.no_grad():
         r = _forward_views_impl(means3D, shs, colors_precomp, opacities, scales, rotations, cov3D_precomp, (raster_settings,),
-                                forward_only, batched=False, tight_tiles=tight_tiles)
+                                forward_only, batched=False, tight_tiles=tight_tiles, no_median=_no_median)
     P = means3D.shape[0]
     r["views"] = state_views(r["state"], P, int(raster_settings.image_height),
                              int(raster_settings.image_width), r["cap"], forward_only)
diff --git a/lara_amd/renderer.py b/lara_amd/renderer.py
--- a/lara_amd/renderer.py
+++ b/lara_amd/renderer.py
@@ -145,6 +145,8 @@
     def __init__(self, sh_degree=3, white_background=True, radius=1, tight_tiles=None):
         super().__init__()
         self.tight_tiles = (os.environ.get("LARA2DGS_TIGHT_TILES", "1") == "1") if tight_tiles is None else bool(tight_tiles)
+        self.no_median = os.environ.get("LARA2DGS_NO_MEDIAN", "1") == "1"
+        self.last_no_median = None
         self.sh_degree, self.white_background, self.radius = sh_degree, white_background, radius
         self.scaling_activation, self.opacity_activation = torch.exp, torch.sigmoid
         self.rotation_activation = torch.nn.functional.normalize
@@ -206,13 +208,18 @@
     def invalidate_activations(self):
         self._act_key, self._act_val = None, None
 
+    def _skip_median(self, rays, depth_ratio, allmap_escapes=False):
+        self.last_no_median = bool(self.no_median and rays is not None and not allmap_escapes and float(depth_ratio) == 0.0)
+        return self.last_no_median
+
     def render_img(self, cam, rays, centers, shs, opacity, scales, rotations, device, cov3D_precomp=None, prex='',
                    depth_ratio=0.0):
         settings = self._settings(cam, device=device)
         opacity, scales, rotations = self._activated(opacity, scales, rotations)
         screenspace_points = self._zero_means2D(centers)
         rendered_image, radii, allmap = rasterize_gaussians(centers, screenspace_points, shs, None, opacity, scales, rotations,
-                                                            cov3D_precomp, settings, tight_tiles=self.tight_tiles)
+                                                            cov3D_precomp, settings, tight_tiles=self.tight_tiles,
+                                                            _no_median=self._skip_median(rays, depth_ratio))
         if rays is None:
             return rendered_image.clamp(0, 1)
         rot = cam.world_view_transform[:3, :3].T
@@ -221,7 +228,8 @@
                 f"depth_normal{prex}": dnorm, f"rend_dist{prex}": rdist}
 
     def render_views(self, cams, rays, centers, shs, opacity, scales, rotations, device, bg_colors=None,
-                     cov3D_precomp=None, prex='', depth_ratio=0.0, concat=False, into=None, raster_out=None, subset_of=None):
+                     cov3D_precomp=None, prex='', depth_ratio=0.0, concat=False, into=None, raster_out=None, subset_of=None,
+                     color_out=None):
         n = len(cams)
         if torch.is_tensor(bg_colors) and bg_colors.dim() == 2 and not (
                 bg_colors.dtype == torch.float32 and bg_colors.stride() == (4, 1) and bg_colors.data_ptr() % 16 == 0):
@@ -231,9 +239,12 @@
         opacity, scales, rotations = self._activated(opacity, scales, rotations)
         color, radii, allmap = rasterize_gaussians_views(settings, centers, self._zero_means2D(centers), opacity, shs=shs,
                                                          scales=scales, rotations=rotations, cov3D_precomp=cov3D_precomp,
-                                                         subset_of=subset_of, tight_tiles=self.tight_tiles)
+                                                         subset_of=subset_of, tight_tiles=self.tight_tiles,
+                                                         _no_median=self._skip_median(rays, depth_ratio, raster_out is not None))
         if raster_out is not None:
             raster_out.append((color, radii, allmap))
+        if color_out is not None:
+            color_out.append(color)
         if concat and rays is not None:
             rots = torch.stack([cam.world_view_transform[:3, :3] for cam in cams]).transpose(1, 2)
             rays_t = rays if torch.is_tensor(rays) else torch.stack(list(rays))
```

Result: no change. 954.5 (median of 4 runs) (+1.0%).
